# carlobaldassi/gimp-lqr-plugin

Hardware: AMD Instinct MI355X
Metric: Mseams*pixels/sec on 4K RGBA (higher is better)
Workload: dtype f32; 1 GPU; batch4k: 64 x 3840x2160 RGBA per GPU, resize to 3640x2160 (200 vertical seams each), side-switch 2; images_per_gpu=64, width=3840, height=2160, new_width=3640, new_height=2160, parallelism=images sharded i mod N, no data-path collective, streams_per_gpu=1

## Files before the change

gimp-lqr-plugin_amd/csrc/k_oneoff.hip:

```cpp
#include "lqr_common.h"
#include "lqr_kernels.h"

__global__ __launch_bounds__(256) void k_vs_commit(const DevCarver *cs, int w0, int h0, int wc0, int n_seams, int first_level,
                                                    int finish)
{
    const GCarver c = gview(cs[blockIdx.y]);
    extern __shared__ int smi[];
    int *xs = smi;
    int *lvl = smi + vsc_lvl_off(n_seams);
    __shared__ int s_wave[4];
    const int y = blockIdx.x, tid = threadIdx.x;
    for (int k = tid; k < n_seams; k += 256) xs[k] = c.seam_log[(size_t) k * h0 + y];
    for (int i = tid; i < wc0; i += 256) lvl[i] = 0;
    __syncthreads();
    for (int k = tid; k < n_seams; k += 256) {
        int pz = xs[k];
        for (int j = k - 1; j >= 0; j--) if (xs[j] <= pz) pz++;
        lvl[pz] = first_level + k;
    }
    __syncthreads();
    gi32 *vrow = c.vs + (size_t) y * w0;
    int carry = 0;
    for (int base = 0; base < w0; base += 256) {
        int col = base + tid;
        bool z = (col < w0) && (vrow[col] == 0);
        int total;
        int rank = carry + block_rank_256(z, s_wave, total);
        if (z) {
            int l = lvl[rank];
            if (l == 0 && finish) l = w0;
            if (l) vrow[col] = l;
        }
        carry += total;
    }
}

template <bool DEEP>
__global__ __launch_bounds__(256) void k_inflate(const InflateDev *jobs, int w0, int w1, int l, int max_level, int *dev_err)
{
    __shared__ int s_wave[4];
    extern __shared__ unsigned s_seen[];
    const int n_levels = l - max_level + 1, lvl0 = 2 * max_level - 1;
    for (int i = threadIdx.x; i < (n_levels + 31) / 32; i += 256) s_seen[i] = 0u;
    __syncthreads();
    bool twice = false;
    const InflateDev j = jobs[blockIdx.y];
    const uint8_t *rgb = j.rgb;
    const int32_t *vs = j.vs;
    const float *bias = j.bias, *rig = j.rig;
    uint8_t *nrgb = j.nrgb;
    int32_t *nvs = j.nvs;
    float *nbias = j.nbias, *nrig = j.nrig;
    const int ch = j.ch;
    const int y = blockIdx.x, tid = threadIdx.x;
    const int32_t *vrow = vs + (size_t) y * w0;
    const size_t ri = (size_t) y * w0, ro = (size_t) y * w1;
    int carry = 0;
    for (int base = 0; base < w0; base += 256) {
        int col = base + tid;
        int v = (col < w0) ? vrow[col] : 0;
        bool dup = (col < w0) && v != 0 && v <= l + max_level - 1 && v >= 2 * max_level - 1;
        if (dup) twice |= (atomicOr(&s_seen[(v - lvl0) >> 5], 1u << ((v - lvl0) & 31)) >> ((v - lvl0) & 31)) & 1u;
        int total;
        int rank = carry + block_rank_256(dup, s_wave, total);
        if (col < w0) {
            int z = col + rank;
            int left = col > 0 ? col - 1 : col;
            if (dup) {
                BasePx<DEEP>::avg(nrgb + (ro + z) * ch, rgb + (ri + left) * ch, rgb + (ri + col) * ch, ch, j.depth);
                if (nbias) nbias[ro + z] = __fmul_rn(__fadd_rn(bias[ri + left], bias[ri + col]), 0.5f);
                if (nrig) nrig[ro + z] = __fmul_rn(__fadd_rn(rig[ri + left], rig[ri + col]), 0.5f);
                if (nvs) nvs[ro + z] = l - v + max_level;
                z++;
            }
            BasePx<DEEP>::move(nrgb + (ro + z) * ch, rgb + (ri + col) * ch, ch);
            if (nbias) nbias[ro + z] = bias[ri + col];
            if (nrig) nrig[ro + z] = rig[ri + col];
            if (nvs) nvs[ro + z] = v ? v + l - max_level + 1 : 0;
        }
        carry += total;
    }
    if (dev_err && (twice || (tid == 0 && carry != n_levels))) dev_fail(dev_err, DEVERR_LEVELS);
}

__global__ __launch_bounds__(256) void k_vmap_check(const int32_t *map, int len, int depth, int *dev_err)
{
    extern __shared__ unsigned s_seen[];
    __shared__ int s_cnt;
    const int tid = threadIdx.x;
    for (int i = tid; i < (depth + 31) / 32; i += 256) s_seen[i] = 0u;
    if (tid == 0) s_cnt = 0;
    __syncthreads();
    const int32_t *row = map + (size_t) blockIdx.x * len;
    bool bad = false;
    int cnt = 0;
    for (int x = tid; x < len; x += 256) {
        const int v = row[x];
        if (v < 0 || v > depth) bad = true;
        else if (v) { bad |= (atomicOr(&s_seen[(v - 1) >> 5], 1u << ((v - 1) & 31)) >> ((v - 1) & 31)) & 1u; cnt++; }
    }
    for (int o = 32; o > 0; o >>= 1) cnt += __shfl_down(cnt, o);
    if ((tid & 63) == 0) atomicAdd(&s_cnt, cnt);
    __syncthreads();
    if (bad || (tid == 0 && s_cnt != depth)) dev_fail(dev_err, DEVERR_VMAP);
}

__global__ __launch_bounds__(256) void k_vmap_check_t(const int32_t *map, int32_t *out, int width, int height, int depth, int *dev_err)
{
    extern __shared__ unsigned s_seen[];
    __shared__ int32_t tile[VT_LINES][33];
    __shared__ int s_cnt[VT_LINES];
    const int tid = threadIdx.x, words = (depth + 31) / 32;
    const int col0 = blockIdx.x * VT_LINES;
    for (int i = tid; i < VT_LINES * words; i += 256) s_seen[i] = 0u;
    if (tid < VT_LINES) s_cnt[tid] = 0;
    bool bad = false;
    for (int row0 = 0; row0 < height; row0 += 32) {
        __syncthreads();
        for (int i = tid; i < VT_LINES * 32; i += 256) {
            const int r = i / VT_LINES, c = i % VT_LINES;
            if (row0 + r < height && col0 + c < width) tile[c][r] = map[(size_t) (row0 + r) * width + col0 + c];
        }
        __syncthreads();
        for (int i = tid; i < VT_LINES * 32; i += 256) {
            const int c = i / 32, r = i % 32;
            if (row0 + r < height && col0 + c < width) {
                const int v = tile[c][r];
                out[(size_t) (col0 + c) * height + row0 + r] = v;
                if (v < 0 || v > depth) bad = true;
                else if (v) {
                    bad |= (atomicOr(&s_seen[c * words + ((v - 1) >> 5)], 1u << ((v - 1) & 31)) >> ((v - 1) & 31)) & 1u;
                    atomicAdd(&s_cnt[c], 1);
                }
            }
        }
    }
    __syncthreads();
    if (tid < VT_LINES && col0 + tid < width && s_cnt[tid] != depth) bad = true;
    if (bad) dev_fail(dev_err, DEVERR_VMAP);
}

__global__ __launch_bounds__(256) void k_seam_check(const DevCarver *cs, int h, int wc0, int n_seams, int delta, int *dev_err)
{
    const GCarver c = gview_phys(cs[blockIdx.y]);
    const int y = blockIdx.x * 256 + threadIdx.x;
    if (y >= h) return;
    bool bad = false;
    for (int k = 0; k < n_seams; k++) {
        const int x = c.seam_log[(size_t) k * h + y];
        bad |= (x < 0) || (x >= wc0 - k);
        if (y > 0) { const int xu = c.seam_log[(size_t) k * h + y - 1]; bad |= (x - xu > delta) || (xu - x > delta); }
    }
    if (bad) dev_fail(dev_err, DEVERR_SEAMLOG);
}

__global__ __launch_bounds__(256) void k_vs_rollback(const DevCarver *cs, size_t n, int first_level, int finish_level)
{
    const GCarver c = gview_phys(cs[blockIdx.y]);
    for (size_t i = (size_t) blockIdx.x * 256 + threadIdx.x; i < n; i += (size_t) gridDim.x * 256) {
        const int v = c.vs[i];
        if (v >= first_level || (finish_level > 0 && v == finish_level)) c.vs[i] = 0;
    }
}

__global__ void k_inject(const DevCarver *cs, int what, int h, int w0, int log_index, int first_level)
{
    const GCarver c = gview_phys(cs[0]);
// ... 146 lines not shown
```

gimp-lqr-plugin_amd/csrc/lqr_kernels.h:

```cpp
#pragma once
#include "lqr_common.h"
#include "lqr_pixel.h"


template <class FORM> __global__ void k_wk_init(const DevCarver *cs, int w, int h, int stride, typename FORM::Arg a);
template <class FORM> __global__ __launch_bounds__(256) void k_wk_init_visible(const DevCarver *cs, int w0, int h, int stride, typename FORM::Arg a);
#define K_EMAP_FORMS(X) X(0, false) X(1, false) X(2, false) X(3, false) X(4, false) X(5, false) X(6, false) X(0, true) X(1, true) X(2, true) X(6, true)
#define K_EMAP_UPDATE_NT_FORMS(X, ...) X(12, __VA_ARGS__) X(36, __VA_ARGS__) X(68, __VA_ARGS__)
template <int NRG, bool VALUE> __global__ void k_emap_full(const DevCarver *cs, DpK p, int w, int h, int stride);
#define K_WK_INIT_EMAP_FORMS(X) X(0) X(1) X(2) X(3) X(4) X(5) X(6)
template <int NRG> __global__ __launch_bounds__(256) void k_wk_init_emap(const DevCarver *cs, DpK p, int w, int h, int stride);
__global__ void k_mask_add(float *plane, int w0, const uint8_t *mask, int channels, int mw, int x0, int y0, int x1, int y1,
                           int nx, int ny, int transposed, int is_rig, int bias_factor);
template <int NRG, int EU_NT, bool VALUE> __global__ __launch_bounds__(64) void k_emap_update(const DevCarver *cs, DpK p, int w, int h, int stride, int k, int epoch);
template <bool VALUE> __global__ __launch_bounds__(256) void k_frozen_catchup(const DevCarver *cs, int from, int to, int w_from, int h, int stride);

__global__ __launch_bounds__(VPATH_THREADS) void k_vpath(const DevCarver *cs, int w, int h, int stride, int lr, int delta, int log_index, int moved_unit);
#define K_VPATH1_FORMS(X) X(1) X(2) X(3) X(4) X(5) X(6) X(7)
#define K_VP_FORMS(X) K_VPATH1_FORMS(X) X(8) X(9) X(10)
template <int DELTA> __global__ __launch_bounds__(VPATH_THREADS) void k_vpath1(const DevCarver *cs, int w, int h, int stride, int lr, int log_index, int moved_unit);
unsigned long long *lqr_moved_bytes_dev(void);

template <int DELTA> __global__ __launch_bounds__(256) void k_vp_maps(const DevCarver *cs, int w, int h, int stride);
template <int DELTA> __global__ __launch_bounds__(VPATH_THREADS) void k_vp_solve(const DevCarver *cs, int w, int h, int stride, int lr, int log_index, int moved_unit);

__global__ __launch_bounds__(256) void k_carve(const DevCarver *cs, int w, int h, int stride, int delta, int move_dp);
#define K_CARVE_E_FORMS(X) X(0) X(1) X(2) X(3) X(4) X(5) X(6)
template <int NRG> __global__ __launch_bounds__(256) void k_carve_e(const DevCarver *cs, DpK p, int w, int h, int stride, int move_dp, int k, int epoch, int line);
#define K_CARVE_U_FORMS(X) X(0) X(1) X(2) X(3) X(4) X(5) X(6)
template <int NRG> __global__ __launch_bounds__(256) void k_carve_u(const DevCarver *cs, DpK p, int w, int h, int stride, int move_dp, int k, int epoch, int n, int line);
#define K_CARVE_V_DELTAS(X) X(1) X(2)
#define K_CARVE_V_FORMS(X) X(0, 1) X(1, 1) X(2, 1) X(3, 1) X(4, 1) X(5, 1) X(6, 1) X(0, 2) X(1, 2) X(2, 2) X(3, 2) X(4, 2) X(5, 2) X(6, 2)
template <int NRG, int DELTA> __global__ __launch_bounds__(256) __attribute__((amdgpu_waves_per_eu(5))) void k_carve_v(const DevCarver *cs, DpK p, int w, int h, int stride, int lr, int move_dp, int k, int epoch, int n,
                                                                                  int moved_unit, unsigned tag, unsigned long long *list, unsigned long long *moved_bytes, int *dev_err, int line);

#define K_DP_SWEEP_PXT_FORMS(X) X(1) X(2) X(4) X(8) X(16)
#define K_LR_RIG_FORMS(X) X(false, false) X(false, true) X(true, false) X(true, true)
template <int PXT, bool UPDATE, int NTH = DP_THREADS> __global__ __launch_bounds__(NTH) void k_dp_sweep(const DevCarver *cs, DpK p, int w, int h, int stride, int lr);
__global__ __launch_bounds__(64) void k_band_update(const DevCarver *cs, DpK p, int w, int h, int stride, int lr);
template <int PXL, int NW, int R, bool LR, bool RIG> __global__ __launch_bounds__(64 * NW) void k_band_update_mw(const DevCarver *cs, DpK p, int w, int h, int stride);
template <int NW, bool LR, bool RIG> __global__ __launch_bounds__(128 * NW) void k_band_update_tw(const DevCarver *cs, DpK p, int w, int h, int stride, int *dev_err);

template <bool LR, bool RIG> __global__ __launch_bounds__(64) void k_dp_tile(const DevCarver *cs, DpK p, int w, int h, int stride, int y0);
#define K_DP_TILE_P_FORMS_D(X, LR, UPD, D) X(GENERAL, 2, LR, false, UPD, D, false, 16) X(GENERAL, 2, LR, true, UPD, D, false, 16) X(GENERAL, 2, LR, true, UPD, D, true, 16)
#define K_DP_TILE_P_FORMS_W(X, LR, UPD, D) X(GENERAL, 2, LR, true, UPD, D, false, 16) X(GENERAL, 2, LR, true, UPD, D, true, 16)
#define K_DP_TILE_P_FORMS_LR(X, LR, UPD) \
    X(PX4, 4, LR, false, UPD, 1, false, 16) X(PX4, 4, LR, true, UPD, 1, false, 16) X(PLAIN, 2, LR, false, UPD, 1, false, 16) X(PLAIN, 2, LR, true, UPD, 1, false, 16) \
    X(GENERAL, 2, LR, true, UPD, 1, true, 16) K_DP_TILE_P_FORMS_D(X, LR, UPD, 2) K_DP_TILE_P_FORMS_D(X, LR, UPD, 3) K_DP_TILE_P_FORMS_D(X, LR, UPD, 4) \
    K_DP_TILE_P_FORMS_W(X, LR, UPD, 5) K_DP_TILE_P_FORMS_W(X, LR, UPD, 6) K_DP_TILE_P_FORMS_W(X, LR, UPD, 7) K_DP_TILE_P_FORMS_W(X, LR, UPD, 8) K_DP_TILE_P_FORMS_W(X, LR, UPD, 9) K_DP_TILE_P_FORMS_W(X, LR, UPD, 10)
#define K_DP_TILE_P_FORMS_24(X, UPD) X(PLAIN, 2, false, false, UPD, 1, false, 24) X(PLAIN, 2, false, true, UPD, 1, false, 24) X(PLAIN, 2, true, false, UPD, 1, false, 24) X(PLAIN, 2, true, true, UPD, 1, false, 24)
#define K_DP_TILE_P_FORMS(X) K_DP_TILE_P_FORMS_LR(X, false, false) K_DP_TILE_P_FORMS_LR(X, false, true) K_DP_TILE_P_FORMS_LR(X, true, false) K_DP_TILE_P_FORMS_LR(X, true, true) \
    K_DP_TILE_P_FORMS_24(X, false) K_DP_TILE_P_FORMS_24(X, true)
template <int PX, bool LR, bool RIG, bool UPDATE, int DELTA = 1, bool RIGM = false, int HLN = 16>
__global__ __launch_bounds__(64 * DPP_W) void k_dp_tile_p(DevCarver *cs, DpK p, int w, int h, int stride, unsigned long long *exch, int epoch, int *dev_err);

#define K_BAND_LEVELS_FORMS_D(X, LR, D) X(LR, false, D, false) X(LR, true, D, false) X(LR, true, D, true)
#define K_BAND_LEVELS_FORMS_W(X, LR, D) X(LR, true, D, false) X(LR, true, D, true)
#define K_BAND_LEVELS_FORMS_LR(X, LR) K_BAND_LEVELS_FORMS_D(X, LR, 1) K_BAND_LEVELS_FORMS_D(X, LR, 2) K_BAND_LEVELS_FORMS_D(X, LR, 3) K_BAND_LEVELS_FORMS_D(X, LR, 4) \
    K_BAND_LEVELS_FORMS_W(X, LR, 5) K_BAND_LEVELS_FORMS_W(X, LR, 6) K_BAND_LEVELS_FORMS_W(X, LR, 7) K_BAND_LEVELS_FORMS_W(X, LR, 8) K_BAND_LEVELS_FORMS_W(X, LR, 9) K_BAND_LEVELS_FORMS_W(X, LR, 10)
#define K_BAND_LEVELS_FORMS(X) K_BAND_LEVELS_FORMS_LR(X, false) K_BAND_LEVELS_FORMS_LR(X, true)
template <bool LR, bool RIG, int DELTA, bool RIGM>
__global__ __launch_bounds__(128) __attribute__((amdgpu_waves_per_eu(2, 2))) void k_band_levels(DevCarver *cs, DpK p, int w, int h, int stride, unsigned long long *exch, int epoch, int *dev_err, int P, int n_img, int store_rows);

#define K_BAND_LEVELS2_FORMS(X) X(false, false) X(false, true) X(true, false) X(true, true)
template <bool LR, bool RIG>
__global__ __launch_bounds__(256) __attribute__((amdgpu_waves_per_eu(2, 2))) void k_band_levels2(DevCarver *cs, DpK p, int w, int h, int stride, unsigned long long *exch, int epoch, int *dev_err, int P, int n_img, int store_rows);
void lqr_levels_report_rows(int on);
void lqr_levels2_debug(int v);
int lqr_levels2_stats(unsigned long long *out, int reset);

__global__ __launch_bounds__(256) void k_vs_commit(const DevCarver *cs, int w0, int h0, int wc0, int n_seams, int first_level, int finish);
template <bool DEEP> __global__ __launch_bounds__(256) void k_inflate(const InflateDev *jobs, int w0, int w1, int l, int max_level, int *dev_err);
__global__ __launch_bounds__(256) void k_vmap_check(const int32_t *map, int len, int depth, int *dev_err);
__global__ __launch_bounds__(256) void k_vmap_check_t(const int32_t *map, int32_t *out, int width, int height, int depth, int *dev_err);
__global__ __launch_bounds__(256) void k_seam_check(const DevCarver *cs, int h, int wc0, int n_seams, int delta, int *dev_err);
__global__ __launch_bounds__(256) void k_vs_rollback(const DevCarver *cs, size_t n, int first_level, int finish_level);
__global__ void k_inject(const DevCarver *cs, int what, int h, int w0, int log_index, int first_level);
template <bool DEEP> __global__ __launch_bounds__(256) void k_compact(const uint8_t *rgb, const int32_t *vs, const float *bias, const float *rig,
                                                  uint8_t *nrgb, float *nbias, float *nrig, int32_t *nvmap, int w0, int w, int ch, int level, int depth);
template <bool DEEP> __global__ __launch_bounds__(256) void k_compact_jobs(const InflateDev *jobs, int w0, int w, int level);
__global__ void k_transpose(const InflateDev *jobs, int w, int h);
__global__ void k_transpose_px(const InflateDev *jobs, int w, int h);
__global__ __launch_bounds__(256) void k_mask_line_max(const uint8_t *mask, int channels, int width, int a0, int b0, int line_len, int direction, int *out);

#define K_COMPACT_SIZES_FORMS(X) X(false) X(true)
#define K_TRANSPOSE_SIZES_FORMS(X) X(false) X(true)
template <bool DEEP> __global__ __launch_bounds__(256) void k_compact_sizes(const uint8_t *rgb, const int32_t *vs, const SizeJob *jobs, int n_jobs, int w0, int bytes);
template <bool WIDE> __global__ __launch_bounds__(256) void k_transpose_sizes(const SizeJob *jobs, int h, int bytes);

#define K_FWD_INIT_FORMS(X) X(0) X(1) X(2) X(3)
#define K_FWD_SEAM_FORMS(X) X(1) X(2) X(4) X(8) X(16)
template <int DEPTH> __global__ __launch_bounds__(256) void k_fwd_init(const FwdJob *jobs, int L, int H, int fw0, int strided, DeepRead rd, int w_start, int orientation);
template <int PXT> __global__ __launch_bounds__(FWD_THREADS) void k_fwd_seam(const FwdJob *jobs, int wc, int L, int H);
__global__ __launch_bounds__(FWD_REMOVE_THREADS) void k_fwd_remove(const FwdJob *jobs, int wc, int L, int H, int level, int orientation);

#define K_CLIP_SEAM_FORMS(X) X(1) X(2) X(4) X(8) X(16)
__global__ __launch_bounds__(CLIPFWD_FOLD_THREADS) void k_clip_fold(const FwdJob *jobs, const float *in, int first, int count, int last, int L, int H, int fw0, int strided,
                                                                   int w_start, float temporal, float *cost, float *pm);
template <int PXT> __global__ __launch_bounds__(FWD_THREADS) void k_clip_seam(const float *cost, int8_t *choice, int32_t *seam, int wc, int L, int H);
__global__ __launch_bounds__(FWD_REMOVE_THREADS) void k_clip_remove(float *cost, uint16_t *pos, const int32_t *seam, int32_t *map, int wc, int L, int H, int level, int orientation);
__global__ __launch_bounds__(CLIPFWD_REFRESH_THREADS) void k_clip_refresh(const float *in, int n, float *cost, const uint16_t *pos, const int32_t *seam, int wn, int L, int H);

#define K_STATIC_FOLD_FORMS(X) X(0, 0, true) X(1, 0, true) X(2, 0, true) X(6, 0, true) X(0, 0, false) X(1, 0, false) X(2, 0, false) X(6, 0, false) \
    X(0, 1, false) X(1, 1, false) X(2, 1, false) X(6, 1, false) X(0, 2, false) X(1, 2, false) X(2, 2, false) X(6, 2, false) \
    X(0, 3, false) X(1, 3, false) X(2, 3, false) X(6, 3, false)
template <int NRG, int DEPTH, bool PACKED>
__global__ __launch_bounds__(STATIC_THREADS) void k_static_fold(const StaticFrame *frames, int count, int first, int W, int H, int transposed, int orientation, DeepRead rd,
                                                     float alpha, float *s_plane, float *t_plane, float *i_plane, float *e_out);

__global__ __launch_bounds__(DISCARD_THREADS) void k_discard_line(const float *bias, const int32_t *vs, int w0, float thr, int level, int depth, int *res);
__global__ __launch_bounds__(DISCARD_THREADS) void k_discard_cross(const float *bias, const int32_t *vs, int w0, int h0, float thr, int level, int depth,
                                                                 int *partial, int *res);
__global__ __launch_bounds__(DISCARD_THREADS) void k_discard_rank(const float *bias, const int32_t *vs, int w0, int w, float thr, int level, int depth, int *col,
                                                                int *res);
__global__ __launch_bounds__(DISCARD_THREADS) void k_discard_fold(const int *partial, int w0, int tiles, int *res);

template <class T> __global__ __launch_bounds__(256) void k_mask_add_f(float *plane, int w0, const T *mask, int mw, int x0, int y0, int x1, int y1, int nx, int ny,
                                                                       int transposed, int is_rig, int bias_factor);
__global__ __launch_bounds__(256) void k_mask_scatter(float *plane, const int *index, const double *value, size_t n, int is_rig);
__global__ __launch_bounds__(256) void k_plane_transpose(const float *plane, float *out, int w0, int h0);

template <bool PIC> __global__ __launch_bounds__(256) void k_energy_range(const DevCarver *cs, int w, int h, int stride, float *partials);
__global__ __launch_bounds__(256) void k_energy_plane(const DevCarver *cs, int w, int h, int stride, int transposed, int normalised,
                                                      const float *partials, int n_partials, float *out);
#define K_ENERGY_OUT_FORMS_T(X, T) X(T, 0) X(T, 1) X(T, 2) X(T, 3)
#define K_ENERGY_OUT_FORMS(X) K_ENERGY_OUT_FORMS_T(X, 0) K_ENERGY_OUT_FORMS_T(X, 1) K_ENERGY_OUT_FORMS_T(X, 2) K_ENERGY_OUT_FORMS_T(X, 3) K_ENERGY_OUT_FORMS_T(X, 4) K_ENERGY_OUT_FORMS_T(X, 5) K_ENERGY_OUT_FORMS_T(X, 6)
template <int TYPE, int DEPTH> __global__ __launch_bounds__(256) void k_energy_out(const DevCarver *cs, int w, int h, int stride, int transposed,
                                                                                    const float *partials, int n_partials, uint8_t *out);
```

gimp-lqr-plugin_amd/csrc/lqr_shim.hip:

```cpp
#include "lqr_common.h"
#include "lqr_kernels.h"
#include "lqr_own.h"
#include "lqr_pool.h"
#include "lqr_stage.h"
#include <atomic>
#include <memory>
#include <dirent.h>

static thread_local std::string g_err;
static int g_device = -1;

static int *g_dev_err_host = nullptr;
static int *g_dev_err = nullptr;

#define HIPCK_VOID(expr) do { hipError_t e__ = (expr); if (e__ != hipSuccess) { g_err = std::string(#expr) + ": " + hipGetErrorString(e__); (void) hipGetLastError(); } } while (0)
#define HIPCK(expr)                                                                   \
    do {                                                                              \
        hipError_t e__ = (expr);                                                      \
        if (e__ != hipSuccess) {                                                      \
            g_err = std::string(#expr) + ": " + hipGetErrorString(e__);               \
            (void) hipGetLastError();                                                 \
            return (e__ == hipErrorOutOfMemory) ? LQRHIP_ENOMEM : LQRHIP_EHIP;        \
        }                                                                             \
    } while (0)

static PlanKnobs g_knobs;
static PlanDevice g_dev;

namespace {
struct WorkingPlanes {
    DevBuf<uint32_t> pix;
    DevBuf<float> en, m, m2, bias, rig;
    DevBuf<int8_t> least, least2;
    DevBuf<int32_t> seam_x, seam_log, flags;
    DevBuf<int8_t> vp_map, vp_path;
};
}
struct __attribute__((visibility("hidden"))) LqrHipCarver {
    int ch = 0;
    int depth = 0;
    int luma = 0;
    int mode = RD_RGB, alpha = -1, black = -1;
    int pix_deep = 0;
    int w0 = 0, h0 = 0;
    DevBuf<uint8_t> rgb0;
    DevBuf<int32_t> vs;
    DevBuf<float> bias0, rig0;
    int active = 0;
    int stride = 0, wk_h = 0;
    WorkingPlanes wk;
    int log_cap = 0, log_h = 0;
    int frozen_epoch = 0;
    int owed_to = 0, owed_w = 0, owed_h = 0;
    LqrHipCarver *root = nullptr;
    std::vector<LqrHipCarver *> aux;
    LqrHipBatch *batch = nullptr;
};

static inline size_t px_bytes(const LqrHipCarver *c) { return (size_t) c->ch << (c->depth == 0 ? 0 : c->depth == 1 ? 1 : c->depth == 2 ? 2 : 3); }
static inline int32_t *vs_of(const LqrHipCarver *c) { return (c->root ? c->root : c)->vs; }

namespace {
struct PlaneJob {
    LqrHipCarver *c;
    DevBuf<uint8_t> nrgb;
    DevBuf<float> nbias, nrig;
};
}
struct PlaneJobs {
    std::vector<PlaneJob> jobs;
    std::vector<DevBuf<int32_t>> new_vs;
    std::vector<InflateDev> dev;
    DevBuf<InflateDev> d_dev;
    size_t n_narrow = 0;
    int add(LqrHipCarver *c, const int32_t *vs_old, int32_t *nvs, size_t n1)
    {
        jobs.push_back(PlaneJob{c, {}, {}, {}});
        PlaneJob &j = jobs.back();
        int rc = j.nrgb.alloc(n1 * px_bytes(c), "&j.nrgb");
        if (!rc && c->bias0) rc = j.nbias.alloc(n1, "&j.nbias");
        if (!rc && c->rig0) rc = j.nrig.alloc(n1, "&j.nrig");
        if (rc) return rc;
        dev.push_back(InflateDev{c->rgb0, vs_old, c->bias0, c->rig0, j.nrgb, nvs, j.nbias, j.nrig, (int) px_bytes(c), c->depth});
        return 0;
    }
    int stage(hipStream_t s, bool by_width)
    {
        n_narrow = std::stable_partition(dev.begin(), dev.end(), [&](const InflateDev &d) { return d.ch <= 4 && (by_width || d.depth == 0); }) - dev.begin();
        int rc = d_dev.alloc(dev.size(), "&d_dev");
        if (rc) return rc;
        HIPCK(hipMemcpyAsync(d_dev, dev.data(), dev.size() * sizeof(InflateDev), hipMemcpyHostToDevice, s));
        return 0;
    }
    size_t n_wide() const { return dev.size() - n_narrow; }
    const InflateDev *d_wide() const { return d_dev + n_narrow; }
};
static void commit(PlaneJobs &pj)
{
    for (auto &j : pj.jobs) {
        j.c->rgb0 = std::move(j.nrgb);
        if (j.nbias) j.c->bias0 = std::move(j.nbias);
        if (j.nrig) j.c->rig0 = std::move(j.nrig);
    }
}

struct PendingInflate { PlaneJobs pj; int kind = 0 , w1 = 0, h1 = 0; };

struct LqrHipBatch {
    std::vector<LqrHipCarver *> cs;
    DevCarver *d_desc = nullptr;
    size_t desc_cap = 0;
    hipStream_t stream = nullptr;
    DevBuf<unsigned long long> exch;
    int exch_ntiles = 0, exch_n = 0, exch_px = 0;
    int tile_epoch = 0;
    DevBuf<unsigned long long> wlist;
    unsigned wlist_launches = 0;
    bool dirty = true;
    int shared_n = 1;
    bool shared = false;
    bool safe = false;
    std::unique_ptr<PendingInflate> pending_inflate;
};
static bool g_no_spin = false;

struct ProfRec {
    std::vector<std::pair<hipEvent_t, hipEvent_t>> ev;
    double bytes = 0;
};
static int g_prof = 0;
static std::map<std::string, ProfRec> g_profrec;
static hipStream_t g_stream0 = nullptr;
static unsigned long long g_census[LQRHIP_CENSUS_SLOTS];
#define CENSUS(slot) (g_census[(slot)]++)
extern "C" int lqrhip_launch_census(unsigned long long *out, int n, int reset)
{
// ... 216 lines not shown
        const unsigned hw = std::thread::hardware_concurrency();
        return new StageRing(dev, STAGE_SLOTS, (size_t) 4 << 20, hw >= 16 ? 8 : hw >= 4 ? (int) hw / 2 : 1);
    }();
    return *ring;
}
static int h2d_staged(void *dst, const void *src, size_t bytes) { return stage_ring().upload(dst, src, bytes); }
static int d2h_staged(void *dst, const void *src, size_t bytes) { return stage_ring().download(dst, src, bytes); }

static inline bool reads_value(const LqrHipCarver *c)
{
    if (c->depth != 0 || c->ch > 4 || (c->mode != RD_GREY && c->mode != RD_RGB)) return true;
    return c->black >= 0 || c->alpha != (c->ch == 2 ? 1 : c->ch == 4 ? 3 : -1);
}
static inline DeepRead deep_read(const LqrHipCarver *c) { return DeepRead{c->ch, c->mode, c->alpha, c->black, c->luma}; }
template <class F> static inline void with_form(const LqrHipCarver *c, F f)
{
    if (reads_value(c)) f(std::true_type{}); else f(std::false_type{});
}
constexpr int plane_nrg(bool value, int nrg) { return value && nrg >= 3 && nrg <= 5 ? nrg - 3 : nrg; }
static inline int nrg_index(int nrg_func) { return nrg_func >= 0 && nrg_func <= 5 ? nrg_func : 6; }
static int no_form(const char *family) { g_err = std::string(family) + ": no instantiation for the parameters asked for"; return LQRHIP_EARG; }
#define LISTED_CASE_(N) if (v__ == N) { f__(std::integral_constant<int, N>{}); return true; }
#define with_listed(LIST, v, f) [&](int v__, auto f__) { LIST(LISTED_CASE_) return false; }(v, f)
static void default_read(LqrHipCarver *c)
{
    c->mode = c->ch <= 2 ? RD_GREY : c->ch <= 4 ? RD_RGB : c->ch == 5 ? RD_CMYK : RD_CUSTOM;
    c->alpha = c->ch == 2 ? 1 : c->ch == 4 ? 3 : c->ch == 5 ? 4 : -1;
    c->black = c->ch == 5 ? 3 : -1;
}

static int batch_sync_of(LqrHipCarver *c)
{
    LqrHipCarver *r = c->root ? c->root : c;
    if (r->batch) HIPCK(hipStreamSynchronize(r->batch->stream));
    return 0;
}

extern "C" LqrHipCarver *lqrhip_carver_create_ext(const void *rgb, int w, int h, int channels, int depth)
{
    if (depth < 0 || depth > 3 || channels < 1 || channels > LQRHIP_MAX_CHANNELS) { g_err = "unsupported colour depth / channels"; return nullptr; }
    if (lqrhip_init() < 0) return nullptr;
    LqrHipCarver *c = new LqrHipCarver();
    c->ch = channels; c->depth = depth; c->w0 = w; c->h0 = h;
    default_read(c);
    const size_t n = (size_t) w * h, bytes = n * px_bytes(c);
    if (c->rgb0.alloc(bytes, "&c->rgb0") || c->vs.alloc(n, "&c->vs")) { lqrhip_carver_destroy(c); return nullptr; }
    if (hipMemsetAsync(c->vs, 0, n * sizeof(int32_t), g_stream0) != hipSuccess || h2d_staged(c->rgb0, rgb, bytes) != 0) {
        g_err = "upload failed";
        lqrhip_carver_destroy(c);
        return nullptr;
    }
    return c;
}

extern "C" LqrHipCarver *lqrhip_carver_create(const unsigned char *rgb, int w, int h, int channels)
{
    return lqrhip_carver_create_ext(rgb, w, h, channels, 0);
}

extern "C" int lqrhip_carver_set_read_luma(LqrHipCarver *c, int luma)
{
    const int changed = reads_value(c) && (luma != 0) != (c->luma != 0);
    c->luma = luma != 0;
    return changed;
}

extern "C" int lqrhip_carver_set_read(LqrHipCarver *c, int image_type, int alpha, int black)
{
    static const int mode_of[8] = {RD_RGB, RD_RGB, RD_GREY, RD_GREY, RD_CMY, RD_CMYK, RD_CMYK, RD_CUSTOM};
    if (image_type < 0 || image_type > 7 || alpha >= c->ch || black >= c->ch) return LQRHIP_EARG;
    const bool was = reads_value(c);
    const int mode = mode_of[image_type], a = alpha < 0 ? -1 : alpha, k = black < 0 ? -1 : black;
    const bool differs = mode != c->mode || a != c->alpha || k != c->black;
    c->mode = mode; c->alpha = a; c->black = k;
    return (differs && (was || reads_value(c))) ? 1 : 0;
}

static inline void drop_catchup(LqrHipCarver *c)
{
    c->owed_to = 0; c->owed_w = 0; c->owed_h = 0;
    c->frozen_epoch = 0;
}

static void free_working(LqrHipCarver *c)
{
    c->wk = WorkingPlanes();
    c->log_cap = 0; c->log_h = 0;
    drop_catchup(c);
}

extern "C" void lqrhip_carver_destroy(LqrHipCarver *c)
{
    if (!c) return;
    {
        LqrHipCarver *r = c->root ? c->root : c;
        if (r->batch && r->batch->stream) (void) hipStreamSynchronize(r->batch->stream);
        if (c->batch && c->batch != r->batch && c->batch->stream) (void) hipStreamSynchronize(c->batch->stream);
        if (g_stream0) (void) hipStreamSynchronize(g_stream0);
        (void) hipGetLastError();
    }
    delete c;
}

extern "C" int lqrhip_carver_attach(LqrHipCarver *root, LqrHipCarver *aux)
{
    if (root->w0 != aux->w0 || root->h0 != aux->h0) return LQRHIP_EARG;
    aux->vs.reset();
    aux->root = root;
    root->aux.push_back(aux);
    if (root->batch) root->batch->dirty = true;
    return 0;
}

static int ensure_working(LqrHipCarver *c, int w, int h)
{
    int stride = plane_stride(w);
    bool need_bias = c->bias0 != nullptr, need_rig = c->rig0 != nullptr;
    const int deep = reads_value(c) ? 1 : 0;
    WorkingPlanes &k = c->wk;
    if (k.pix && c->stride == stride && c->wk_h == h && (!!k.bias == need_bias) && (!!k.rig == need_rig) && c->pix_deep == deep) return 0;
    free_working(c);
    c->stride = 0; c->wk_h = 0;
    size_t n = plane_elems(stride, h);
    const size_t npix = deep ? 2 * n : n;
    int rc;
    if ((rc = k.pix.alloc(npix, "&c->pix")) || (rc = k.en.alloc(n, "&c->en")) || (rc = k.m.alloc(n, "&c->m")) || (rc = k.least.alloc(n, "&c->least")) ||
        (rc = k.seam_x.alloc(seam_x_elems(h), "&c->seam_x")) || (rc = k.flags.alloc((size_t) FLAG_WORDS, "&c->flags")) ||
        (need_bias && (rc = k.bias.alloc(n, "&c->bias"))) || (need_rig && (rc = k.rig.alloc(n, "&c->rig")))) {
        free_working(c);
        return rc;
    }
    hipError_t e = hipMemsetAsync(k.least, 0, n, g_stream0);
    if (e == hipSuccess) e = hipMemsetAsync(k.m, 0, n * sizeof(float), g_stream0);
    if (e == hipSuccess) e = hipMemsetAsync(k.en, 0, n * sizeof(float), g_stream0);
    if (e == hipSuccess) e = hipMemsetAsync(k.pix, 0, npix * sizeof(uint32_t), g_stream0);
    if (e == hipSuccess) e = hipMemsetAsync(k.flags, 0, (size_t) FLAG_WORDS * sizeof(int32_t), g_stream0);
    if (e == hipSuccess) e = hipStreamSynchronize(g_stream0);
    if (e != hipSuccess) { free_working(c); HIPCK(e); }
    c->stride = stride; c->wk_h = h; c->pix_deep = deep;
    if (c->batch) c->batch->dirty = true;
    return 0;
}

static int ensure_log(LqrHipCarver *c, int n_seams, int h)
{
    if (c->wk.seam_log && c->log_cap >= n_seams && c->log_h == h) return 0;
    int rc = c->wk.seam_log.alloc(seam_log_elems(n_seams, h), "&c->seam_log");
    if (rc) return rc;
    c->log_cap = n_seams; c->log_h = h;
    if (c->batch) c->batch->dirty = true;
    return 0;
}

extern "C" int lqrhip_carver_activate(LqrHipCarver *c)
{
    c->active = 1;
    return ensure_working(c, c->w0, c->h0);
}

extern "C" int lqrhip_mask_plane_ensure(LqrHipCarver *c, int is_rigmask)
{
    DevBuf<float> &plane = is_rigmask ? c->rig0 : c->bias0;
    if (plane) return 0;
    int rc = batch_sync_of(c);
    if (rc) return rc;
    const size_t n = (size_t) c->w0 * c->h0;
    if ((rc = plane.alloc(n, "plane"))) return rc;
    hipError_t e = dzero(plane, n * sizeof(float));
    if (e != hipSuccess) { plane.reset(); HIPCK(e); }
    if (c->batch) c->batch->dirty = true;
    return 0;
}

extern "C" int lqrhip_mask_add(LqrHipCarver *c, const unsigned char *mask, int channels, int width, int height, int x_off,
                               int y_off, int transposed, int is_rigmask, int bias_factor)
{
    int rc = batch_sync_of(c);
    if (rc) return rc;
    if ((rc = lqrhip_mask_plane_ensure(c, is_rigmask))) return rc;
    float *plane = is_rigmask ? c->rig0 : c->bias0;
    const MaskClip k = mask_clip(c->w0, c->h0, width, height, x_off, y_off, transposed);
    if (k.nx <= 0 || k.ny <= 0) return 0;
    const size_t mbytes = (size_t) width * height * channels;
    Scratch tmp(g_stream0);
    uint8_t *dmask = tmp.get<uint8_t>(mbytes, "&dmask", rc);
    if (rc || (rc = h2d_staged(dmask, mask, mbytes))) return rc;
    dim3 grid(tiles_of(k.nx, 256), k.ny);
    hipLaunchKernelGGL(k_mask_add, grid, dim3(256), 0, g_stream0, plane, c->w0, dmask, channels, width, k.x0, k.y0, k.x1, k.y1, k.nx, k.ny,
                       transposed, is_rigmask, bias_factor);
    HIPCK(hipGetLastError());
    HIPCK(hipStreamSynchronize(g_stream0));
    tmp.done();
    return 0;
}

extern "C" int lqrhip_mask_add_f(LqrHipCarver *c, const void *mask, int depth, int on_device, int width, int height, int x_off, int y_off,
                                 int transposed, int is_rigmask, int bias_factor)
{
    if ((depth != 2 && depth != 3) || !mask || width < 1 || height < 1) { g_err = "mask: float or double values, at least 1 x 1"; return LQRHIP_EARG; }
    int rc = batch_sync_of(c);
    if (rc) return rc;
    if ((rc = lqrhip_mask_plane_ensure(c, is_rigmask))) return rc;
    float *plane = is_rigmask ? c->rig0 : c->bias0;
    const MaskClip k = mask_clip(c->w0, c->h0, width, height, x_off, y_off, transposed);
    if (k.nx <= 0 || k.ny <= 0) return 0;
    const size_t mbytes = (size_t) width * height * (depth == 2 ? sizeof(float) : sizeof(double));
    Scratch tmp(g_stream0);
    const void *src = mask;
    if (!on_device) {
        uint8_t *staged = tmp.get<uint8_t>(mbytes, "&staged", rc);
        if (rc || (rc = h2d_staged(staged, mask, mbytes))) return rc;
        src = staged;
    }
    dim3 grid(tiles_of(k.nx, 256), k.ny);
    if (depth == 2)
        hipLaunchKernelGGL(k_mask_add_f<float>, grid, dim3(256), 0, g_stream0, plane, c->w0, (const float *) src, width, k.x0, k.y0, k.x1, k.y1, k.nx, k.ny,
                           transposed, is_rigmask, bias_factor);
    else
        hipLaunchKernelGGL(k_mask_add_f<double>, grid, dim3(256), 0, g_stream0, plane, c->w0, (const double *) src, width, k.x0, k.y0, k.x1, k.y1, k.nx, k.ny,
                           transposed, is_rigmask, bias_factor);
    HIPCK(hipGetLastError());
    HIPCK(hipStreamSynchronize(g_stream0));
    tmp.done();
    return 0;
}

static unsigned long long g_mask_flushes = 0;
extern "C" unsigned long long lqrhip_debug_mask_flushes(void) { return g_mask_flushes; }

extern "C" int lqrhip_mask_scatter(LqrHipCarver *c, int is_rigmask, const int *index, const double *value, const size_t *start, int buckets)
{
    if (buckets < 1 || start[buckets] == 0) return 0;
    int rc = batch_sync_of(c);
    if (rc) return rc;
    if ((rc = lqrhip_mask_plane_ensure(c, is_rigmask))) return rc;
    float *plane = is_rigmask ? c->rig0 : c->bias0;
    const size_t n = start[buckets];
    Scratch tmp(g_stream0);
    int *dindex = tmp.get<int>(n, "&dindex", rc);
    if (rc) return rc;
    double *dvalue = tmp.get<double>(n, "&dvalue", rc);
    if (rc || (rc = h2d_staged(dindex, index, n * sizeof(int))) || (rc = h2d_staged(dvalue, value, n * sizeof(double)))) return rc;
    for (int b = 0; b < buckets; b++) {
        const size_t nb = start[b + 1] - start[b];
        if (!nb) continue;
        hipLaunchKernelGGL(k_mask_scatter, dim3((unsigned) blocks_of(nb, 256)), dim3(256), 0, g_stream0, plane, dindex + start[b], dvalue + start[b],
                           nb, is_rigmask);
        HIPCK(hipGetLastError());
        g_mask_flushes++;
    }
    HIPCK(hipStreamSynchronize(g_stream0));
    tmp.done();
    return 0;
}

extern "C" int lqrhip_mask_clear(LqrHipCarver *c, int is_rigmask)
{
    DevBuf<float> &plane = is_rigmask ? c->rig0 : c->bias0;
    if (!plane) return 0;
    int rc = batch_sync_of(c);
    if (rc) return rc;
    HIPCK(hipStreamSynchronize(g_stream0));
    plane.reset();
    if (c->batch) c->batch->dirty = true;
    return 0;
}

extern "C" int lqrhip_read_mask_plane(LqrHipCarver *c, int is_rigmask, int transposed, float *out)
{
    int rc = batch_sync_of(c);
    if (rc) return rc;
    const size_t n = (size_t) c->w0 * c->h0;
    const float *plane = is_rigmask ? c->rig0 : c->bias0;
    if (!plane) { memset(out, 0, n * sizeof(float)); return 0; }
    if (!transposed) return d2h_staged(out, plane, n * sizeof(float));
    Scratch tmp(g_stream0);
    float *t = tmp.get<float>(n, "&t", rc);
    if (rc) return rc;
    hipLaunchKernelGGL(k_plane_transpose, dim3(tiles_of(c->w0, 16), tiles_of(c->h0, 16)), dim3(256), 0, g_stream0, plane, t, c->w0, c->h0);
    hipError_t e = hipGetLastError();
    if (e != hipSuccess) { g_err = std::string("k_plane_transpose: ") + hipGetErrorString(e); return LQRHIP_EHIP; }
    if ((rc = d2h_staged(out, t, n * sizeof(float)))) return rc;
    (void) hipStreamSynchronize(g_stream0);
    tmp.done();
    return 0;
}

extern "C" void lqrhip_set_sub_batches(int n) { g_knobs.sub_batches = n > 0 ? n : 0; }
extern "C" int lqrhip_sub_batches(int n)
{
    const char *q = getenv("GPU_MAX_HW_QUEUES");
    g_dev.hw_queues = q ? atoi(q) : 0;
    return plan_streams(g_knobs, g_dev, n);
}

extern "C" void lqrhip_batch_set_shared(LqrHipBatch *b, int shared) { b->shared = shared != 0; b->shared_n = shared > 1 ? shared : 1; }
extern "C" void lqrhip_batch_set_safe(LqrHipBatch *b, int safe) { b->safe = safe != 0; if (safe) g_fault_stats[6]++; }

static const size_t MAX_PARKED = 4;
static std::vector<hipStream_t> g_parked_streams;
static unsigned long long g_fixed_stats[3];
static std::multimap<size_t, DevCarver *> g_parked_desc;
extern "C" void lqrhip_debug_fixedcost(unsigned long long out4[4], int reset)
{
    out4[0] = g_parked_streams.size();
    for (int i = 0; i < 3; i++) out4[i + 1] = g_fixed_stats[i];
    if (reset) memset(g_fixed_stats, 0, sizeof g_fixed_stats);
}
static void unpark_all(void)
{
    for (hipStream_t s : g_parked_streams) (void) hipStreamDestroy(s);
    g_parked_streams.clear();
    for (auto &kv : g_parked_desc) (void) hipFree(kv.second);
    g_parked_desc.clear();
}

extern "C" LqrHipBatch *lqrhip_batch_create(LqrHipCarver **carvers, int n)
{
    if (lqrhip_init() < 0 || n <= 0) return nullptr;
    LqrHipBatch *b = new LqrHipBatch();
    for (int i = 0; i < n; i++) {
        b->cs.push_back(carvers[i]);
        carvers[i]->batch = b;
    }
    hipError_t e = hipSuccess;
    if (!g_parked_streams.empty()) { b->stream = g_parked_streams.back(); g_parked_streams.pop_back(); g_fixed_stats[0]++; }
    else e = hipStreamCreateWithFlags(&b->stream, hipStreamNonBlocking);
    if (e == hipSuccess) {
        auto it = g_parked_desc.lower_bound((size_t) n);
        if (it != g_parked_desc.end()) { b->d_desc = it->second; b->desc_cap = it->first; g_parked_desc.erase(it); }
        else if ((e = hipMalloc((void **) &b->d_desc, sizeof(DevCarver) * n)) == hipSuccess) b->desc_cap = (size_t) n;
    }
    if (e != hipSuccess) {
        g_err = "batch_create failed";
        (void) hipGetLastError();
        if (b->stream) (void) hipStreamDestroy(b->stream);
        for (auto *c : b->cs) if (c->batch == b) c->batch = nullptr;
        delete b;
        return nullptr;
    }
    g_live_batches.push_back(b);
    return b;
}

static void invalidate_all_batches(void)
{
    for (auto *b : g_live_batches) { b->exch_ntiles = 0; b->dirty = true; }
}

extern "C" void lqrhip_batch_abort(LqrHipBatch *b)
{
    if (!b) return;
    (void) hipStreamSynchronize(b->stream);
    (void) hipGetLastError();
// ... 59 lines not shown

struct ProfScope {
    ProfRec *rec = nullptr;
    hipEvent_t e0 = nullptr, e1 = nullptr;
    hipStream_t s;
    ProfScope(const char *name, hipStream_t stream, double bytes) : s(stream)
    {
        if (!g_prof || (g_prof == 2 && strcmp(name, "carve") != 0)) return;
        rec = &g_profrec[name];
        rec->bytes += bytes;
        (void) hipEventCreate(&e0); (void) hipEventCreate(&e1);
        (void) hipEventRecord(e0, s);
    }
    ~ProfScope()
    {
        if (!rec) return;
        (void) hipEventRecord(e1, s);
        rec->ev.emplace_back(e0, e1);
    }
};

extern "C" void lqrhip_prof_enable(int on) { g_prof = on; }
extern "C" void lqrhip_prof_reset(void)
{
    for (auto &kv : g_profrec) for (auto &e : kv.second.ev) { (void) hipEventDestroy(e.first); (void) hipEventDestroy(e.second); }
    g_profrec.clear();
}
extern "C" int lqrhip_prof_get(const char *kernel, double *ms_total, long long *launches, double *bytes_total)
{
    auto it = g_profrec.find(kernel);
    *ms_total = 0; *launches = 0; *bytes_total = 0;
    if (it == g_profrec.end()) return 0;
    (void) hipDeviceSynchronize();
    for (auto &e : it->second.ev) {
        float ms = 0;
        if (hipEventElapsedTime(&ms, e.first, e.second) == hipSuccess) *ms_total += ms;
    }
    *launches = (long long) it->second.ev.size();
    *bytes_total = it->second.bytes;
    return 0;
}

extern "C" int lqrhip_prof_get_union(const char *kernel, double *ms_union)
{
    *ms_union = 0;
    auto it = g_profrec.find(kernel);
    if (it == g_profrec.end() || it->second.ev.empty()) return 0;
    (void) hipDeviceSynchronize();
    const hipEvent_t base = it->second.ev[0].first;
    std::vector<std::pair<float, float>> iv;
    for (auto &e : it->second.ev) {
        float a = 0, b = 0;
        if (hipEventElapsedTime(&a, base, e.first) != hipSuccess) { (void) hipGetLastError(); float t = 0; if (hipEventElapsedTime(&t, e.first, base) == hipSuccess) a = -t; else (void) hipGetLastError(); }
        if (hipEventElapsedTime(&b, base, e.second) != hipSuccess) { (void) hipGetLastError(); float t = 0; if (hipEventElapsedTime(&t, e.second, base) == hipSuccess) b = -t; else (void) hipGetLastError(); }
        iv.emplace_back(a, b);
    }
    std::sort(iv.begin(), iv.end());
    float end = -1e30f;
    for (auto &p : iv) {
        if (p.first > end) { *ms_union += p.second - p.first; end = p.second; }
        else if (p.second > end) { *ms_union += p.second - end; end = p.second; }
    }
    return 0;
}

static int pay_catchup(LqrHipBatch *b);
static int wk_init_prepare(LqrHipBatch *b)
{
    LqrHipCarver *c0 = b->cs[0];
    int w = c0->w0, h = c0->h0, rc;
    for (auto *c : b->cs) {
        if (c->w0 != w || c->h0 != h || c->ch != c0->ch || c->depth != c0->depth || c->luma != c0->luma || c->mode != c0->mode ||
            c->alpha != c0->alpha || c->black != c0->black)
            return LQRHIP_EARG;
        if ((rc = ensure_working(c, w, h))) return rc;
    }
    if ((rc = batch_upload(b))) return rc;
    for (auto *c : b->cs) drop_catchup(c);
    return 0;
}
extern "C" int lqrhip_wk_init(LqrHipBatch *b, int from_visible)
{
    LqrHipCarver *c0 = b->cs[0];
    int w = c0->w0, h = c0->h0, rc;
    if ((rc = wk_init_prepare(b))) return rc;
    const dim3 grid(tiles_of(c0->stride, 256), h, (unsigned) b->cs.size()), grid_v(h, (unsigned) b->cs.size());
#define LAUNCH_WK(FORM, arg) do { if (from_visible) hipLaunchKernelGGL(k_wk_init_visible<FORM>, grid_v, dim3(256), 0, b->stream, b->d_desc, w, h, c0->stride, arg); \
                                  else hipLaunchKernelGGL(k_wk_init<FORM>, grid, dim3(256), 0, b->stream, b->d_desc, w, h, c0->stride, arg); } while (0)
    if (!reads_value(c0)) LAUNCH_WK(PixPacked, c0->ch);
    else if (c0->depth == 0) LAUNCH_WK(PixValue<0>, deep_read(c0));
    else if (c0->depth == 1) LAUNCH_WK(PixValue<1>, deep_read(c0));
    else if (c0->depth == 2) LAUNCH_WK(PixValue<2>, deep_read(c0));
    else LAUNCH_WK(PixValue<3>, deep_read(c0));
#undef LAUNCH_WK
    HIPCK(hipGetLastError());
    return 0;
}

extern "C" int lqrhip_emap_build(LqrHipBatch *b, const LqrHipDpParams *p, int w, int h)
{
    int rc;
    if ((rc = pay_catchup(b))) return rc;
    if ((rc = batch_upload(b))) return rc;
    LqrHipCarver *c0 = b->cs[0];
    dim3 grid(tiles_of(w, 256), h, (unsigned) b->cs.size());
    DpK k = make_dpk(p, c0->ch);
    const bool value = reads_value(c0);
    const int nrg = plane_nrg(value, nrg_index(p->nrg_func));
#define CASE(N, V) if (nrg == N && value == V) hipLaunchKernelGGL((k_emap_full<N, V>), grid, dim3(256), 0, b->stream, b->d_desc, k, w, h, c0->stride); else
    K_EMAP_FORMS(CASE) return no_form("k_emap_full");
#undef CASE
    HIPCK(hipGetLastError());
    return 0;
}

extern "C" int lqrhip_wk_init_emap(LqrHipBatch *b, const LqrHipDpParams *p, int w, int h)
{
    LqrHipCarver *c0 = b->cs[0];
    int rc;
    if (reads_value(c0) || w != c0->w0 || h != c0->h0) return (rc = lqrhip_wk_init(b, 0)) ? rc : lqrhip_emap_build(b, p, w, h);
    if ((rc = wk_init_prepare(b))) return rc;
    const dim3 grid(tiles_of(tiles_of(c0->stride, 4), 256), h, (unsigned) b->cs.size());
    DpK k = make_dpk(p, c0->ch);
    const int nrg = nrg_index(p->nrg_func);
#define CASE(N) if (nrg == N) hipLaunchKernelGGL(k_wk_init_emap<N>, grid, dim3(256), 0, b->stream, b->d_desc, k, w, h, c0->stride); else
    K_WK_INIT_EMAP_FORMS(CASE) return no_form("k_wk_init_emap");
#undef CASE
    HIPCK(hipGetLastError());
    return 0;
}

extern "C" int lqrhip_energy_out(LqrHipBatch *b, int w, int h, int transposed, int form, int depth, int image_type, void *out, int on_device)
{
    static const int channels_of[7] = {3, 4, 1, 2, 3, 4, 5};
    if (b->cs.size() != 1 || !out || w < 1 || h < 1 || form < 0 || form > 2) { g_err = "energy read-out: one carver, a buffer, form 0 .. 2"; return LQRHIP_EARG; }
    if (form != 2) { depth = 2; image_type = 2; }
    if (depth < 0 || depth > 3 || image_type < 0 || image_type > 6) { g_err = "energy read-out: depth 0 .. 3, image type 0 .. 6"; return LQRHIP_EARG; }
    int rc;
    if ((rc = batch_upload(b))) return rc;
    LqrHipCarver *c0 = b->cs[0];
    if (!c0->wk.en) return LQRHIP_EARG;
    const size_t bytes = (size_t) w * h * channels_of[image_type] << depth;
    const int chunks = (w + EO_CHUNK - 1) / EO_CHUNK;
    const int n_partials = form ? (int) std::min((long long) EO_MAX_PARTIALS, (long long) h * chunks) : 0;
    Scratch tmp(b->stream);
    float *partials = form ? tmp.get<float>((size_t) 2 * n_partials, "&partials", rc) : nullptr;
    if (rc) return rc;
    uint8_t *staged = on_device ? nullptr : tmp.get<uint8_t>(bytes, "&staged", rc);
    if (rc) return rc;
    uint8_t *dst = on_device ? (uint8_t *) out : staged;
    {
        ProfScope prof("energy_out", b->stream, (double) w * h * sizeof(float) * (form ? 2 : 1) + (double) bytes);
        if (form == 1) hipLaunchKernelGGL(k_energy_range<false>, dim3(n_partials), dim3(256), 0, b->stream, b->d_desc, w, h, c0->stride, partials);
        if (form == 2) hipLaunchKernelGGL(k_energy_range<true>, dim3(n_partials), dim3(256), 0, b->stream, b->d_desc, w, h, c0->stride, partials);
        const int W = transposed ? h : w, H = transposed ? w : h;
        const dim3 grid((W + EO_TILE - 1) / EO_TILE, (H + EO_TILE - 1) / EO_TILE);
#define CASE(T, D) if (image_type == T && depth == D) hipLaunchKernelGGL((k_energy_out<T, D>), grid, dim3(256), 0, b->stream, b->d_desc, w, h, c0->stride, transposed, partials, n_partials, dst); else
        if (form != 2)
            hipLaunchKernelGGL(k_energy_plane, grid, dim3(256), 0, b->stream, b->d_desc, w, h, c0->stride, transposed, form, partials, n_partials, (float *) dst);
        else K_ENERGY_OUT_FORMS(CASE) return no_form("k_energy_out");
#undef CASE
    }
    hipError_t e = hipGetLastError();
    if (e == hipSuccess) e = hipStreamSynchronize(b->stream);
    if (e != hipSuccess) { g_err = std::string("energy read-out: ") + hipGetErrorString(e); (void) hipGetLastError(); return LQRHIP_EHIP; }
    if ((rc = check_dev_error())) return rc;
    if (!on_device && (rc = d2h_staged(out, staged, bytes))) return rc;
    tmp.done();
    return 0;
}

static int launch_dp_tiled(LqrHipBatch *b, const DpK &k, int w, int h, int lr)
{
    LqrHipCarver *c0 = b->cs[0];
    const dim3 grid(tiles_of(w, DPT_OWN), (unsigned) b->cs.size());
    for (int y0 = 0; y0 < h; y0 += DPT_ROWS) {
        CENSUS(LQRHIP_CENSUS_DP_TILE);
#define CASE(LRV, RIGV) if ((lr != 0) == LRV && (k.use_rig != 0) == RIGV) hipLaunchKernelGGL((k_dp_tile<LRV, RIGV>), grid, dim3(64), 0, b->stream, b->d_desc, k, w, h, c0->stride, y0); else
        K_LR_RIG_FORMS(CASE) return no_form("k_dp_tile");
#undef CASE
    }
    HIPCK(hipGetLastError());
    return 0;
}

extern "C" void lqrhip_set_vpath_mode(int mode, int par_max) { g_knobs.vpath_mode = mode; if (par_max > 0) g_knobs.vpath_par_max = par_max; }
extern "C" void lqrhip_set_sweep_threads(int n) { g_knobs.sweep_threads = n == 256 ? 256 : DP_THREADS; }
extern "C" void lqrhip_set_carve_fused(int max_images) { g_knobs.carve_fused = max_images == 1 ? 4 : max_images < 0 ? 0 : max_images; }
extern "C" void lqrhip_set_carve_beside(int mode) { g_knobs.carve_beside = mode < 0 ? -1 : mode ? 1 : 0; }
static unsigned long long g_carve_beside_launches;
extern "C" unsigned long long lqrhip_carve_beside_launches(int reset)
{
    const unsigned long long v = g_carve_beside_launches;
    if (reset) g_carve_beside_launches = 0;
    return v;
}
extern "C" void lqrhip_set_backtrack_beside(int mode) { g_knobs.backtrack_beside = mode < 0 ? -1 : mode ? 1 : 0; }
static unsigned long long g_backtrack_beside_launches;
extern "C" unsigned long long lqrhip_backtrack_beside_launches(int reset)
{
    const unsigned long long v = g_backtrack_beside_launches;
    if (reset) g_backtrack_beside_launches = 0;
// ... 321 lines not shown
        if (int rc = launch_band_levels(b, k, wnew, h, leftright_next, s.levels_P, s.levels_wg_slots, s.levels_store, v.rigm)) return rc;
    } else if (s.band == LQRHIP_CENSUS_BAND_TW) {
        ProfScope ps("band_update", b->stream, 0);
        CENSUS(LQRHIP_CENSUS_BAND_TW);
#define CASE(LRV, RIGV) if ((leftright_next != 0) == LRV && (k.use_rig != 0) == RIGV) hipLaunchKernelGGL((k_band_update_tw<4, LRV, RIGV>), dim3(n), dim3(128 * 4), band_tw_lds(h), b->stream, b->d_desc, k, wnew, h, stride, g_dev_err); else
        K_LR_RIG_FORMS(CASE) return no_form("k_band_update_tw");
#undef CASE
    } else if (s.band == LQRHIP_CENSUS_BAND_MW8 || s.band == LQRHIP_CENSUS_BAND_MW16) {
        ProfScope ps("band_update", b->stream, 0);
        const int nw = s.band == LQRHIP_CENSUS_BAND_MW16 ? 16 : 8;
        CENSUS(nw == 16 ? LQRHIP_CENSUS_BAND_MW16 : LQRHIP_CENSUS_BAND_MW8);
#define CASE_NW(NWV, LRV, RIGV) if (nw == NWV && (leftright_next != 0) == LRV && (k.use_rig != 0) == RIGV) hipLaunchKernelGGL((k_band_update_mw<2, NWV, 8, LRV, RIGV>), dim3(n), dim3(64 * NWV), band_mw_lds(h), b->stream, b->d_desc, k, wnew, h, stride); else
#define CASE(LRV, RIGV) CASE_NW(8, LRV, RIGV) CASE_NW(16, LRV, RIGV)
        K_LR_RIG_FORMS(CASE) return no_form("k_band_update_mw");
#undef CASE
#undef CASE_NW
    } else {
        ProfScope ps("band_update", b->stream, 0);
        CENSUS(LQRHIP_CENSUS_BAND_GENERIC);
        hipLaunchKernelGGL(k_band_update, dim3(n), dim3(64), 0, b->stream, b->d_desc, k, wnew, h, stride, leftright_next);
    }
    ProfScope ps("dp_update", b->stream, 0);
    return launch_dp<true>(b, k, s.dp, v.rigm, wnew, h, leftright_next);
}

static int seam_step_impl(LqrHipBatch *b, const LqrHipDpParams *p, int w, int h, int log_index, int leftright_pick,
                          int full_rebuild, int leftright_next)
{
    int rc;
    LqrHipCarver *c0 = b->cs[0];
    for (auto *c : b->cs)
        if (log_index >= c->log_cap || c->owed_to) return LQRHIP_EARG;
    if ((rc = batch_upload(b))) return rc;
    const PlanBatch pb = plan_batch(b);
    const StepPlan s = plan_seam_step(g_knobs, g_dev, pb, p->delta_x, p->use_rigidity != 0, w, h, full_rebuild != 0, log_index + 1 - c0->frozen_epoch);
    const int wnew = w - 1, move_dp = (wnew > 1 && !full_rebuild) ? 1 : 0;
    const int moved_unit = 2 * (4 + (move_dp ? 5 : 0) + (pb.rigmask ? 4 : 0));
    StepVals v{make_dpk(p, c0->ch), w, h, c0->stride, log_index, leftright_pick, leftright_next, move_dp, moved_unit, c0->frozen_epoch,
               pb.value, pb.rigm(p->use_rigidity != 0), (unsigned) b->cs.size()};
    if ((rc = launch_backtrack(b, s, v)) || (rc = launch_carve(b, s, v))) return rc;
    if (s.dp.form < 0) { HIPCK(hipGetLastError()); return 0; }
    if ((rc = launch_energy(b, s, v))) return rc;
    if (s.full || s.band < 0) {
        ProfScope ps(s.full ? "dp_sweep" : "dp_update_tiled", b->stream, s.full ? 9.0 * wnew * h * v.n : 0);
        rc = s.full ? launch_dp<false>(b, v.k, s.dp, v.rigm, wnew, h, leftright_next) : launch_dp<true>(b, v.k, s.dp, v.rigm, wnew, h, leftright_next);
    } else rc = launch_band(b, s, v);
    if (rc) return rc;
    HIPCK(hipGetLastError());
    return 0;
}

extern "C" int lqrhip_seam_step(LqrHipBatch *b, const LqrHipDpParams *p, int w, int h, int log_index, int leftright_pick,
                                int full_rebuild, int leftright_next)
{
    const int rc = seam_step_impl(b, p, w, h, log_index, leftright_pick, full_rebuild, leftright_next);
    if (rc == 0) inject_after_step(b, h, log_index);
    static const char *dump = getenv("LQRHIP_DUMP");
    if (rc == 0 && dump) {
        static int call = 0;
        LqrHipCarver *c = b->cs[0];
        HIPCK(hipStreamSynchronize(b->stream));
        const size_t np = (size_t) c->stride * h;
        std::vector<int> hdr = {w, h, c->stride, log_index, FLAG_COUNT}, flags(FLAG_COUNT), seam(h);
        std::vector<float> m(np);
        std::vector<int8_t> least(np);
        HIPCK(hipMemcpy(flags.data(), c->wk.flags, FLAG_COUNT * sizeof(int), hipMemcpyDeviceToHost));
        HIPCK(hipMemcpy(seam.data(), c->wk.seam_x, (size_t) h * sizeof(int), hipMemcpyDeviceToHost));
        HIPCK(hipMemcpy(m.data(), c->wk.m, np * sizeof(float), hipMemcpyDeviceToHost));
        HIPCK(hipMemcpy(least.data(), c->wk.least, np, hipMemcpyDeviceToHost));
        char path[512];
        snprintf(path, sizeof path, "%s_%04d.bin", dump, call++);
        if (FILE *f = fopen(path, "wb")) {
            fwrite(hdr.data(), sizeof(int), hdr.size(), f); fwrite(flags.data(), sizeof(int), flags.size(), f);
            fwrite(seam.data(), sizeof(int), seam.size(), f); fwrite(m.data(), sizeof(float), np, f); fwrite(least.data(), 1, np, f);
            fclose(f);
        }
    }
    return rc;
}

extern "C" int lqrhip_seam_log_reserve(LqrHipBatch *b, int n_seams, int h)
{
    int rc;
    if ((rc = pay_catchup(b))) return rc;
    for (auto *c : b->cs) if ((rc = ensure_log(c, n_seams, h))) return rc;
    return 0;
}

extern "C" int lqrhip_vs_commit(LqrHipBatch *b, int w0, int h0, int wc0, int n_seams, int first_level, int finish)
{
    int rc;
    if ((rc = batch_upload(b))) return rc;
    size_t lds = vsc_lds(n_seams, wc0);
    if (lds > VSC_LDS_MAX) { g_err = "vs_commit: session too large for LDS"; return LQRHIP_EARG; }
    if (lds_needs_attr(lds)) {
        HIPCK(hipFuncSetAttribute((const void *) k_vs_commit, hipFuncAttributeMaxDynamicSharedMemorySize, (int) lds));
        CENSUS(LQRHIP_CENSUS_LDS_ATTR_COMMIT);
    }
    hipLaunchKernelGGL(k_vs_commit, dim3(h0, (unsigned) b->cs.size()), dim3(256), lds, b->stream, b->d_desc, w0, h0, wc0, n_seams,
                       first_level, finish);
    HIPCK(hipGetLastError());
    inject_after_commit(b, w0, h0, first_level);
    for (auto *c : b->cs) {
        if (c->frozen_epoch < n_seams) { c->owed_to = n_seams; c->owed_w = wc0 - n_seams; c->owed_h = h0; }
        else drop_catchup(c);
    }
    return 0;
}

static int g_selfcheck = 1, g_recovery = 1;
extern "C" void lqrhip_set_selfcheck(int on) { g_selfcheck = on != 0; }
extern "C" void lqrhip_set_recovery(int on) { g_recovery = on != 0; }
extern "C" int lqrhip_get_recovery(void) { return g_recovery; }
extern "C" int lqrhip_session_check(LqrHipBatch *b, int h, int wc0, int n_seams, int delta_x)
{
    int rc;
    if (!g_selfcheck || n_seams < 1) return 0;
    if ((rc = batch_upload(b))) return rc;
    hipLaunchKernelGGL(k_seam_check, dim3(tiles_of(h, 256), (unsigned) b->cs.size()), dim3(256), 0, b->stream, b->d_desc, h, wc0, n_seams, delta_x, g_dev_err);
    HIPCK(hipGetLastError());
    return 0;
}
extern "C" int lqrhip_session_rollback(LqrHipBatch *b, int w0, int h0, int first_level, int finish)
{
    (void) hipStreamSynchronize(b->stream);
    b->pending_inflate.reset();
    (void) hipGetLastError();
    if (g_dev_err_host) *g_dev_err_host = 0;
    invalidate_all_batches();
    int rc;
    if ((rc = batch_upload(b))) return rc;
    const size_t n = (size_t) w0 * h0;
    hipLaunchKernelGGL(k_vs_rollback, dim3((unsigned) std::min<size_t>(blocks_of(n, 256), 4096), (unsigned) b->cs.size()), dim3(256), 0, b->stream, b->d_desc, n, first_level, finish ? w0 : 0);
    HIPCK(hipGetLastError());
    HIPCK(hipStreamSynchronize(b->stream));
    for (auto *c : b->cs) drop_catchup(c);
    g_fault_stats[4]++;
    return 0;
}
static int g_inject_kind = 0, g_inject_step = 0, g_inject_times = 0;
extern "C" void lqrhip_debug_inject(int kind, int at_step, int times) { g_inject_kind = kind; g_inject_step = at_step; g_inject_times = kind ? std::max(times, 1) : 0; }
static void inject_after_step(LqrHipBatch *b, int h, int log_index)
{
    if (g_inject_times <= 0 || log_index != g_inject_step) return;
    if (g_inject_kind == 1 || g_inject_kind == 2) { *g_dev_err_host = g_inject_kind == 1 ? DEVERR_TILE_TIMEOUT : DEVERR_BAND_PREDICTION; }
    else if (g_inject_kind == 3 || g_inject_kind == 4) hipLaunchKernelGGL(k_inject, dim3(1), dim3(64), 0, b->stream, b->d_desc, g_inject_kind - 3, h, 0, log_index, 0);
    else return;
    g_inject_times--; g_fault_stats[5]++;
}
static void inject_after_commit(LqrHipBatch *b, int w0, int h0, int first_level)
{
    if (g_inject_times <= 0 || (g_inject_kind != 5 && g_inject_kind != 6)) return;
    if (g_inject_step > 0) { g_inject_step--; return; }
    hipLaunchKernelGGL(k_inject, dim3(1), dim3(64), 0, b->stream, b->d_desc, g_inject_kind - 3, h0, w0, 0, first_level);
    g_inject_times--; g_fault_stats[5]++;
}

namespace {
struct Staging {
    LqrHipBatch *b;
    bool keep = false;
    Staging(LqrHipBatch *batch, int kind, int w1, int h1) : b(batch)
    {
        b->pending_inflate.reset(new PendingInflate());
        b->pending_inflate->kind = kind; b->pending_inflate->w1 = w1; b->pending_inflate->h1 = h1;
    }
    ~Staging() { if (!keep) { lqr_stream_wait(b->stream); b->pending_inflate.reset(); } }
    PlaneJobs &jobs() const { return b->pending_inflate->pj; }
    int kept() { keep = true; return 0; }
};
}
static int inflate_stage(LqrHipBatch *b, int w0, int h0, int l, int max_level, const int32_t *levels)
{
    int rc;
    const int w1 = w0 + l - max_level + 1;
    Staging st(b, 0, w1, h0);
    PlaneJobs &pj = st.jobs();
    for (auto *c : b->cs) {
        pj.new_vs.emplace_back();
        DevBuf<int32_t> &nvs = pj.new_vs.back();
        if ((rc = nvs.alloc((size_t) w1 * h0, "&nvs"))) return rc;
        const int32_t *vs = levels ? levels : c->vs.get();
        for (auto *a : c->aux)
            if ((rc = pj.add(a, vs, nullptr, (size_t) w1 * h0))) return rc;
        if ((rc = pj.add(c, vs, nvs, (size_t) w1 * h0))) return rc;
    }
    if ((rc = pj.stage(b->stream, false))) return rc;
    const size_t lds = inflate_lds(l, max_level);
    if (pj.n_narrow)
        hipLaunchKernelGGL(k_inflate<false>, dim3(h0, (unsigned) pj.n_narrow), dim3(256), lds, b->stream, pj.d_dev.get(), w0, w1, l, max_level, g_selfcheck ? g_dev_err : (int *) nullptr);
    if (pj.n_wide())
        hipLaunchKernelGGL(k_inflate<true>, dim3(h0, (unsigned) pj.n_wide()), dim3(256), lds, b->stream, pj.d_wide(), w0, w1, l, max_level, g_selfcheck ? g_dev_err : (int *) nullptr);
    HIPCK(hipGetLastError());
    HIPCK(hipStreamSynchronize(b->stream));
    if ((rc = check_dev_error())) return rc;
    return st.kept();
}
extern "C" int lqrhip_inflate(LqrHipBatch *b, int w0, int h0, int l, int max_level) { return inflate_stage(b, w0, h0, l, max_level, nullptr); }

struct __attribute__((visibility("hidden"))) LqrHipVMap {
    DevBuf<int32_t> own;
    const int32_t *plane = nullptr;
    int len = 0, lines = 0, depth = 0;
};
extern "C" int lqrhip_vmap_stage(const int *map, int on_device, int width, int height, int depth, int orientation, LqrHipVMap **out)
{
    *out = nullptr;
    if (lqrhip_init() < 0) return LQRHIP_EHIP;
    const int len = orientation ? height : width, lines = orientation ? width : height;
    if (!map || width < 1 || height < 1 || (orientation != 0 && orientation != 1) || depth < 1 || depth >= len || depth >= LQRHIP_MAX_FRAME_WIDTH) {
        g_err = "vmap: depth, size or orientation out of range";
        return LQRHIP_EARG;
    }
    int rc;
    const size_t n = (size_t) width * height;
    std::unique_ptr<LqrHipVMap> m(new LqrHipVMap());
    m->len = len; m->lines = lines; m->depth = depth;
    Scratch tmp(g_stream0);
    const int32_t *src = (const int32_t *) map;
    if (!on_device) {
        int32_t *d = orientation ? tmp.get<int32_t>(n, "&vmap_raw", rc) : ((rc = m->own.alloc(n, "&vmap")) ? nullptr : m->own.get());
        if (rc) return rc;
        if ((rc = h2d_staged(d, map, n * sizeof(int32_t)))) return rc;
        src = d;
    }
    if (orientation) {
        if ((rc = m->own.alloc(n, "&vmap_t"))) return rc;
        const size_t lds = vmap_check_t_lds(depth);
        if (vmap_t_needs_attr(lds)) HIPCK(hipFuncSetAttribute((const void *) k_vmap_check_t, hipFuncAttributeMaxDynamicSharedMemorySize, (int) lds));
        hipLaunchKernelGGL(k_vmap_check_t, dim3(vmap_t_blocks(width)), dim3(256), lds, g_stream0, src, m->own.get(), width, height, depth, g_dev_err);
        m->plane = m->own;
    } else {
        hipLaunchKernelGGL(k_vmap_check, dim3(height), dim3(256), vmap_check_lds(depth), g_stream0, src, width, depth, g_dev_err);
        m->plane = src;
    }
    HIPCK(hipGetLastError());
    HIPCK(hipStreamSynchronize(g_stream0));
    tmp.done();
    if (g_dev_err_host && *g_dev_err_host == DEVERR_VMAP) {
        *g_dev_err_host = 0;
        g_err = "vmap: a value outside [0, depth], or a level that is missing or occurs twice in a line";
        return LQRHIP_EMAP;
    }
    if ((rc = check_dev_error())) return rc;
    *out = m.release();
    return 0;
}
extern "C" void lqrhip_vmap_release(LqrHipVMap *m) { delete m; }
extern "C" int lqrhip_vmap_load(LqrHipBatch *b, const LqrHipVMap *m)
{
    if (!m || !m->plane) return LQRHIP_EARG;
    for (auto *c : b->cs)
        if (c->w0 != m->len || c->h0 != m->lines) { g_err = "vmap: the carver's frame is not the map's"; return LQRHIP_EARG; }
    return inflate_stage(b, m->len, m->lines, m->depth, 1, m->plane);
}
extern "C" int lqrhip_planes_commit(LqrHipBatch *b)
{
    PendingInflate *pi = b->pending_inflate.get();
    if (!pi) return LQRHIP_EARG;
    PlaneJobs &pj = pi->pj;
    commit(pj);
    for (auto &j : pj.jobs) { j.c->w0 = pi->w1; j.c->h0 = pi->h1; }
    if (pi->kind != 0)
        for (auto *c : b->cs) drop_catchup(c);
    if (pi->kind != 2) {
        size_t i = 0;
        for (auto *c : b->cs) c->vs = std::move(pj.new_vs[i++]);
    }
    b->dirty = true;
    b->pending_inflate.reset();
    return 0;
}
extern "C" int lqrhip_inflate_commit(LqrHipBatch *b) { return lqrhip_planes_commit(b); }

extern "C" int lqrhip_flatten(LqrHipBatch *b, int w0, int h0, int w, int level)
{
    int rc;
    Staging st(b, 1, w, h0);
    PlaneJobs &pj = st.jobs();
    for (auto *c : b->cs) {
        pj.new_vs.emplace_back();
        DevBuf<int32_t> &nvs = pj.new_vs.back();
        if ((rc = nvs.alloc((size_t) w * h0, "&nvs"))) return rc;
        HIPCK(hipMemsetAsync(nvs, 0, (size_t) w * h0 * sizeof(int32_t), b->stream));
        for (auto *a : c->aux)
            if ((rc = pj.add(a, c->vs, nullptr, (size_t) w * h0))) return rc;
        if ((rc = pj.add(c, c->vs, nullptr, (size_t) w * h0))) return rc;
    }
    if ((rc = pj.stage(b->stream, true))) return rc;
    if (pj.n_narrow)
        hipLaunchKernelGGL(k_compact_jobs<false>, dim3(h0, (unsigned) pj.n_narrow), dim3(256), 0, b->stream, pj.d_dev.get(), w0, w, level);
    if (pj.n_wide())
        hipLaunchKernelGGL(k_compact_jobs<true>, dim3(h0, (unsigned) pj.n_wide()), dim3(256), 0, b->stream, pj.d_wide(), w0, w, level);
    HIPCK(hipGetLastError());
    HIPCK(hipStreamSynchronize(b->stream));
    return st.kept();
}

extern "C" int lqrhip_transpose(LqrHipBatch *b, int w, int h)
{
    int rc;
    Staging st(b, 2, h, w);
    PlaneJobs &pj = st.jobs();
    for (auto *c : b->cs) {
        for (auto *a : c->aux)
            if ((rc = pj.add(a, nullptr, nullptr, (size_t) w * h))) return rc;
        if ((rc = pj.add(c, nullptr, nullptr, (size_t) w * h))) return rc;
        HIPCK(hipMemsetAsync(c->vs, 0, (size_t) w * h * sizeof(int32_t), b->stream));
    }
    if ((rc = pj.stage(b->stream, true))) return rc;
    if (pj.n_narrow)
        hipLaunchKernelGGL(k_transpose, dim3(tiles_of(w, 32), tiles_of(h, 32), (unsigned) pj.n_narrow), dim3(32, 8), 0, b->stream, pj.d_dev.get(), w, h);
    if (pj.n_wide())
        hipLaunchKernelGGL(k_transpose_px, dim3(tiles_of(w, 32), tiles_of(h, 32), (unsigned) pj.n_wide()), dim3(32, 8), 0, b->stream, pj.d_wide(), w, h);
    HIPCK(hipGetLastError());
    HIPCK(hipStreamSynchronize(b->stream));
    return st.kept();
}

static void launch_read_visible(const LqrHipCarver *c, int w0, int h0, int w, int level, uint8_t *d)
{
#define LAUNCH_RV(DEEP) hipLaunchKernelGGL(k_compact<DEEP>, dim3(h0), dim3(256), 0, g_stream0, c->rgb0.get(), vs_of(c), (const float *) nullptr, (const float *) nullptr, \
                                           d, (float *) nullptr, (float *) nullptr, (int32_t *) nullptr, w0, w, (int) px_bytes(c), level, 0)
    if (px_bytes(c) > 4) LAUNCH_RV(true); else LAUNCH_RV(false);
#undef LAUNCH_RV
}
extern "C" int lqrhip_read_visible(LqrHipCarver *c, int w0, int h0, int w, int level, unsigned char *out)
{
    int rc = batch_sync_of(c);
    if (rc) return rc;
    size_t n = (size_t) w * h0 * px_bytes(c);
    Scratch tmp(g_stream0);
    uint8_t *d = tmp.get<uint8_t>(n, "&d", rc);
    if (rc) return rc;
    launch_read_visible(c, w0, h0, w, level, d);
    HIPCK(hipGetLastError());
    if ((rc = d2h_staged(out, d, n))) return rc;
    tmp.done();
    return 0;
}

extern "C" int lqrhip_read_visible_device(LqrHipCarver *c, int w0, int h0, int w, int level, void *device_out)
{
    int rc = batch_sync_of(c);
    if (rc) return rc;
    launch_read_visible(c, w0, h0, w, level, (uint8_t *) device_out);
    HIPCK(hipGetLastError());
    HIPCK(hipStreamSynchronize(g_stream0));
    return 0;
}

static const size_t SZ_SCRATCH_MAX = (size_t) 512 << 20;
extern "C" int lqrhip_read_sizes(LqrHipCarver *c, int w0, int h0, int transposed, const int *levels, int n, void *const *outs, int on_device)
{
    int rc = batch_sync_of(c);
    if (rc) return rc;
    if (n < 1 || !levels || !outs || w0 < 1 || h0 < 1) return LQRHIP_EARG;
    for (int k = 0; k < n; k++)
        if (levels[k] < 1 || levels[k] > w0 || !outs[k]) return LQRHIP_EARG;
    const size_t bytes = px_bytes(c);
    const int planes = (on_device ? 0 : 1) + (transposed ? 1 : 0);
    auto width_of = [&](int k) { return w0 - levels[k] + 1; };
    auto plane_bytes = [&](int k) { return ((size_t) width_of(k) * h0 * bytes + 255) & ~(size_t) 255; };
    struct Chunk { int first, count; };
    std::vector<Chunk> chunks;
    size_t scratch_bytes = 0;
    for (int k = 0; k < n;) {
        size_t used = 0;
        int m = 0;
        while (k + m < n && m < SZ_MAX_JOBS && (m == 0 || used + planes * plane_bytes(k + m) <= SZ_SCRATCH_MAX)) used += planes * plane_bytes(k + m), m++;
        chunks.push_back(Chunk{k, m});
        scratch_bytes = std::max(scratch_bytes, used);
        k += m;
    }
    std::vector<SizeJob> jobs(2 * (size_t) n);
    std::vector<const uint8_t *> result(n);
    Scratch tmp(g_stream0);
    SizeJob *d_jobs = tmp.get<SizeJob>(2 * (size_t) n, "&d_jobs", rc);
    if (rc) return rc;
    uint8_t *scratch = nullptr;
    if (planes) {
        scratch = tmp.get<uint8_t>(scratch_bytes, "&scratch", rc);
        if (rc) return rc;
    }
    for (const Chunk &ch : chunks) {
        size_t at = 0;
        for (int k = ch.first; k < ch.first + ch.count; k++) {
            uint8_t *frame = (uint8_t *) outs[k], *image = (uint8_t *) outs[k];
            if (planes) { frame = scratch + at; at += plane_bytes(k); }
            if (transposed && !on_device) { image = scratch + at; at += plane_bytes(k); }
            jobs[k] = SizeJob{frame, nullptr, levels[k], width_of(k)};
            jobs[n + k] = SizeJob{image, frame, levels[k], width_of(k)};
            result[k] = transposed ? image : frame;
        }
    }
    HIPCK(hipMemcpyAsync(d_jobs, jobs.data(), jobs.size() * sizeof(SizeJob), hipMemcpyHostToDevice, g_stream0));
    for (const Chunk &ch : chunks) {
#define LAUNCH_CS(DEEP) hipLaunchKernelGGL(k_compact_sizes<DEEP>, dim3(h0), dim3(256), 0, g_stream0, (const uint8_t *) c->rgb0.get(), (const int32_t *) vs_of(c), \
                                           (const SizeJob *) (d_jobs + ch.first), ch.count, w0, (int) bytes)
        if (bytes > 4) LAUNCH_CS(true); else LAUNCH_CS(false);
#undef LAUNCH_CS
        CENSUS(LQRHIP_CENSUS_COMPACT_SIZES);
        HIPCK(hipGetLastError());
        if (transposed) {
            int wmax = 0;
            for (int k = ch.first; k < ch.first + ch.count; k++) wmax = std::max(wmax, width_of(k));
            const dim3 grid(tiles_of(wmax, 32), tiles_of(h0, 32), (unsigned) ch.count);
#define LAUNCH_TS(WIDE) hipLaunchKernelGGL(k_transpose_sizes<WIDE>, grid, dim3(256), 0, g_stream0, (const SizeJob *) (d_jobs + n + ch.first), h0, (int) bytes)
            if (bytes > 4) LAUNCH_TS(true); else LAUNCH_TS(false);
#undef LAUNCH_TS
            CENSUS(LQRHIP_CENSUS_TRANSPOSE_SIZES);
            HIPCK(hipGetLastError());
        }
        if (!on_device)
            for (int k = ch.first; k < ch.first + ch.count; k++)
                if ((rc = d2h_staged(outs[k], result[k], (size_t) width_of(k) * h0 * bytes))) return rc;
    }
    HIPCK(hipStreamSynchronize(g_stream0));
    tmp.done();
    return 0;
}

static unsigned long long g_discard_launches[4];
extern "C" void lqrhip_discard_launches(unsigned long long out4[4], int reset)
{
    if (out4) memcpy(out4, g_discard_launches, sizeof g_discard_launches);
    if (reset) memset(g_discard_launches, 0, sizeof g_discard_launches);
}
extern "C" int lqrhip_discard_scan(LqrHipCarver *c, int w0, int h0, int w, int level, int depth, float strength, int which, int *out)
{
    if (!c || c->root || !out || w0 < 1 || h0 < 1 || w < 1 || w > w0 || level < 1 || depth < 0 || !(which & 3) || !(strength >= 0.0f) || c->w0 != w0 || c->h0 != h0) {
        g_err = "discard scan: a root carver in its own base layout, a level, a strength >= 0 and a scan to run";
        return LQRHIP_EARG;
    }
    int rc = batch_sync_of(c);
    if (rc) return rc;
    const bool line = which & LQRHIP_DISCARD_LINE, cross = which & LQRHIP_DISCARD_CROSS;
    memset(out, 0, discard_result_elems() * sizeof(int));
    if (!c->bias0) return 0;
    Scratch tmp(g_stream0);
    int *res = tmp.get<int>(discard_result_elems(), "&res", rc);
    if (rc) return rc;
    const bool ranked = cross && level > 1;
    int *partial = nullptr;
    if (cross) {
        partial = tmp.get<int>(ranked ? discard_rank_elems(w) : discard_partial_elems(w0, h0), "&partial", rc);
        if (rc) return rc;
    }
    HIPCK(hipMemsetAsync(res, 0, discard_result_elems() * sizeof(int), g_stream0));
    if (ranked) HIPCK(hipMemsetAsync(partial, 0, discard_rank_elems(w) * sizeof(int), g_stream0));
    const float thr = -strength;
    const double plane_bytes = 8.0 * w0 * h0;
    if (line) {
        ProfScope ps("discard_line", g_stream0, plane_bytes);
        hipLaunchKernelGGL(k_discard_line, dim3(h0), dim3(DISCARD_THREADS), 0, g_stream0, (const float *) c->bias0.get(), (const int32_t *) c->vs.get(), w0, thr, level,
                           depth, res + discard_result_off(0));
        g_discard_launches[0]++;
        HIPCK(hipGetLastError());
    }
    if (ranked) {
        ProfScope ps("discard_cross", g_stream0, plane_bytes);
        hipLaunchKernelGGL(k_discard_rank, dim3(h0), dim3(DISCARD_THREADS), 0, g_stream0, (const float *) c->bias0.get(), (const int32_t *) c->vs.get(), w0, w, thr, level,
                           depth, partial, res + discard_result_off(1));
        g_discard_launches[2]++;
        HIPCK(hipGetLastError());
        hipLaunchKernelGGL(k_discard_fold, dim3(discard_col_blocks(w)), dim3(DISCARD_THREADS), 0, g_stream0, (const int *) partial, w, 1, res + discard_result_off(1));
        g_discard_launches[3]++;
        HIPCK(hipGetLastError());
    } else if (cross) {
        ProfScope ps("discard_cross", g_stream0, plane_bytes + 8.0 * discard_partial_elems(w0, h0));
        hipLaunchKernelGGL(k_discard_cross, dim3(discard_col_blocks(w0), discard_row_tiles(h0)), dim3(DISCARD_THREADS), 0, g_stream0, (const float *) c->bias0.get(),
                           (const int32_t *) c->vs.get(), w0, h0, thr, level, depth, partial, res + discard_result_off(1));
        g_discard_launches[1]++;
        HIPCK(hipGetLastError());
        hipLaunchKernelGGL(k_discard_fold, dim3(discard_col_blocks(w0)), dim3(DISCARD_THREADS), 0, g_stream0, (const int *) partial, w0, discard_row_tiles(h0),
                           res + discard_result_off(1));
        g_discard_launches[3]++;
        HIPCK(hipGetLastError());
    }
    const int first = line ? 0 : 1, count = line && cross ? 2 : 1;
    if ((rc = d2h_staged(out + discard_result_off(first), res + discard_result_off(first), (size_t) count * DISCARD_WORDS * sizeof(int)))) return rc;
    tmp.done();
    return 0;
}

struct __attribute__((visibility("hidden"))) LqrHipForward {
    struct Planes {
        DevBuf<float> in, p;
        DevBuf<uint16_t> pos;
        DevBuf<int8_t> choice;
        DevBuf<int32_t> seam, map;
    };
    std::vector<Planes> img;
    std::vector<FwdJob> jobs;
    DevBuf<FwdJob> d_jobs;
    hipEvent_t slice_end[2] = {nullptr, nullptr};
    int slices = 0, next_seam = 0;
    int n = 0, L = 0, H = 0, depth = 0, orientation = 0, pxt = 0;
    size_t lds = 0;
    ~LqrHipForward()
    {
        if (g_stream0) (void) hipStreamSynchronize(g_stream0);
        for (hipEvent_t e : slice_end)
            if (e) (void) hipEventDestroy(e);
        (void) hipGetLastError();
    }
};
static std::atomic<unsigned long long> g_forward_launches{0};
extern "C" unsigned long long lqrhip_forward_launches(int reset)
{
    return reset ? g_forward_launches.exchange(0, std::memory_order_relaxed) : g_forward_launches.load(std::memory_order_relaxed);
}
static FwdJob forward_job(const LqrHipCarver *c, const LqrHipForward::Planes &pl, int32_t *map)
{
    return FwdJob{c->rgb0, c->bias0, pl.in, pl.p, pl.pos, pl.choice, pl.seam, map};
}
static int forward_launch_init(const LqrHipCarver *c0, const FwdJob *d_jobs, int n, int L, int H, int strided, int luma, int w_start, int orientation,
                               std::atomic<unsigned long long> &launches = g_forward_launches)
{
    DeepRead rd = deep_read(c0);
    rd.luma = luma != 0;
    const dim3 grid(tiles_of(L, 256), H, (unsigned) n);
#define CASE(D) if (c0->depth == D) hipLaunchKernelGGL(k_fwd_init<D>, grid, dim3(256), 0, g_stream0, d_jobs, L, H, c0->w0, strided, rd, w_start, orientation); else
    K_FWD_INIT_FORMS(CASE) return no_form("k_fwd_init");
#undef CASE
    launches.fetch_add(1, std::memory_order_relaxed);
    HIPCK(hipGetLastError());
    return 0;
}
extern "C" int lqrhip_forward_begin(LqrHipCarver *const *cs, int n, int depth, int orientation, int transposed, int luma, int w_start,
                                    void *const *device_maps, LqrHipForward **out)
{
    if (out) *out = nullptr;
    if (!cs || !out || n < 1 || n > LQRHIP_FORWARD_MAX_LINES || (orientation != 0 && orientation != 1) || w_start < 1) { g_err = "forward map: arguments"; return LQRHIP_EARG; }
    const LqrHipCarver *c0 = cs[0];
    for (int i = 0; i < n; i++) {
        const LqrHipCarver *c = cs[i];
        if (!c || c->root || c->w0 != c0->w0 || c->h0 != c0->h0 || c->ch != c0->ch || c->depth != c0->depth || c->mode != c0->mode ||
            c->alpha != c0->alpha || c->black != c0->black || (device_maps && !device_maps[i])) {
            g_err = "forward map: root carvers of one shape and pixel kind, a map for each";
            return LQRHIP_EARG;
        }
    }
    const int strided = (transposed != 0) != (orientation != 0);
    const int L = strided ? c0->h0 : c0->w0, H = strided ? c0->w0 : c0->h0;
    if (depth < 1 || depth >= L || L > FWD_THREADS * FWD_MAX_PXT || L > LQRHIP_MAX_FRAME_WIDTH || H > LQRHIP_FORWARD_MAX_LINES) {
        g_err = "forward map: 0 < depth < line length <= " + std::to_string(LQRHIP_MAX_FRAME_WIDTH) + ", at most " + std::to_string(LQRHIP_FORWARD_MAX_LINES) + " lines";
        return LQRHIP_EARG;
    }
    int rc;
    for (int i = 0; i < n; i++)
        if ((rc = batch_sync_of(cs[i]))) return rc;
    std::unique_ptr<LqrHipForward> f(new LqrHipForward());
    f->n = n; f->L = L; f->H = H; f->depth = depth; f->orientation = orientation;
    f->pxt = L <= FWD_THREADS ? 1 : L <= 2 * FWD_THREADS ? 2 : L <= 4 * FWD_THREADS ? 4 : L <= 8 * FWD_THREADS ? 8 : 16;
    f->lds = fwd_lds(L);
    const size_t px = (size_t) L * H;
    f->img.resize(n);
    for (int i = 0; i < n; i++) {
        LqrHipForward::Planes &pl = f->img[i];
        if ((rc = pl.in.alloc(px, "&fwd_in")) || (cs[i]->bias0 && (rc = pl.p.alloc(px, "&fwd_p"))) || (rc = pl.pos.alloc(px, "&fwd_pos")) ||
            (rc = pl.choice.alloc(px, "&fwd_choice")) || (rc = pl.seam.alloc((size_t) H, "&fwd_seam")) ||
            (!device_maps && (rc = pl.map.alloc(px, "&fwd_map"))))
            return rc;
        f->jobs.push_back(forward_job(cs[i], pl, device_maps ? (int32_t *) device_maps[i] : pl.map.get()));
    }
    if ((rc = f->d_jobs.alloc((size_t) n, "&fwd_jobs"))) return rc;
    for (hipEvent_t &e : f->slice_end) HIPCK(hipEventCreateWithFlags(&e, hipEventDisableTiming));
    if (lds_needs_attr(f->lds)) {
#define CASE(P) if (f->pxt == P) HIPCK(hipFuncSetAttribute((const void *) k_fwd_seam<P>, hipFuncAttributeMaxDynamicSharedMemorySize, (int) f->lds)); else
        K_FWD_SEAM_FORMS(CASE) return no_form("k_fwd_seam");
#undef CASE
    }
    HIPCK(hipMemcpyAsync(f->d_jobs, f->jobs.data(), (size_t) n * sizeof(FwdJob), hipMemcpyHostToDevice, g_stream0));
    if ((rc = forward_launch_init(c0, f->d_jobs, n, L, H, strided, luma, w_start, orientation))) return rc;
    *out = f.release();
    return 0;
}
extern "C" int lqrhip_forward_seams(LqrHipForward *f, int first_seam, int n_seams)
{
    if (!f || first_seam != f->next_seam || n_seams < 1 || first_seam + n_seams > f->depth) { g_err = "forward map: seams out of order or range"; return LQRHIP_EARG; }
    for (int s = first_seam; s < first_seam + n_seams; s++) {
        const int wc = f->L - s;
#define CASE(P) if (f->pxt == P) hipLaunchKernelGGL(k_fwd_seam<P>, dim3((unsigned) f->n), dim3(FWD_THREADS), f->lds, g_stream0, (const FwdJob *) f->d_jobs.get(), wc, f->L, f->H); else
        K_FWD_SEAM_FORMS(CASE) return no_form("k_fwd_seam");
#undef CASE
        hipLaunchKernelGGL(k_fwd_remove, dim3((unsigned) f->H, (unsigned) f->n), dim3(FWD_REMOVE_THREADS), 0, g_stream0, (const FwdJob *) f->d_jobs.get(), wc, f->L,
                           f->H, s + 1, f->orientation);
        g_forward_launches.fetch_add(2, std::memory_order_relaxed);
        HIPCK(hipGetLastError());
    }
    f->next_seam = first_seam + n_seams;
    HIPCK(hipEventRecord(f->slice_end[f->slices & 1], g_stream0));
    if (f->slices > 0) HIPCK(hipEventSynchronize(f->slice_end[(f->slices - 1) & 1]));
    f->slices++;
    return 0;
}
extern "C" int lqrhip_forward_finish(LqrHipForward *f)
{
    if (!f || f->next_seam != f->depth) { g_err = "forward map: the build is not complete"; return LQRHIP_EARG; }
    HIPCK(hipStreamSynchronize(g_stream0));
    return check_dev_error();
}
extern "C" const int *lqrhip_forward_map(const LqrHipForward *f, int i)
{
    return (f && i >= 0 && i < f->n) ? (const int *) f->jobs[i].map : nullptr;
}
extern "C" int lqrhip_forward_read_map(LqrHipForward *f, int i, int *out)
{
    if (!f || i < 0 || i >= f->n || !out) return LQRHIP_EARG;
    return d2h_staged(out, f->jobs[i].map, (size_t) f->L * f->H * sizeof(int32_t));
}
extern "C" void lqrhip_forward_release(LqrHipForward *f) { delete f; }
extern "C" int lqrhip_forward_intensity(LqrHipCarver *c, int orientation, int transposed, int luma, float *out)
{
    if (!c || c->root || !out || (orientation != 0 && orientation != 1)) return LQRHIP_EARG;
    int rc = batch_sync_of(c);
    if (rc) return rc;
    const int strided = (transposed != 0) != (orientation != 0);
    const int L = strided ? c->h0 : c->w0, H = strided ? c->w0 : c->h0;
    if (L > LQRHIP_MAX_FRAME_WIDTH || H > LQRHIP_FORWARD_MAX_LINES) return LQRHIP_EARG;
    const size_t px = (size_t) L * H;
    Scratch tmp(g_stream0);
    float *in = tmp.get<float>(px, "&fwd_in", rc);
    uint16_t *pos = rc ? nullptr : tmp.get<uint16_t>(px, "&fwd_pos", rc);
    int32_t *map = rc ? nullptr : tmp.get<int32_t>(px, "&fwd_map", rc);
    FwdJob *d_job = rc ? nullptr : tmp.get<FwdJob>(1, "&fwd_jobs", rc);
    if (rc) return rc;
    const FwdJob job{c->rgb0, nullptr, in, nullptr, pos, nullptr, nullptr, map};
    HIPCK(hipMemcpyAsync(d_job, &job, sizeof job, hipMemcpyHostToDevice, g_stream0));
    HIPCK(hipStreamSynchronize(g_stream0));
    if ((rc = forward_launch_init(c, d_job, 1, L, H, strided, luma, 1, orientation))) return rc;
    if ((rc = d2h_staged(out, in, px * sizeof(float)))) return rc;
    tmp.done();
    return 0;
}

struct __attribute__((visibility("hidden"))) LqrHipStatic {
    Scratch tmp{g_stream0};
    std::vector<StaticFrame> frames;
    StaticFrame *d_frames = nullptr;
    float *s = nullptr, *t = nullptr, *ip = nullptr, *e = nullptr;
    int n = 0, W = 0, H = 0, transposed = 0, orientation = 0, nrg = 0, depth = 0, next = 0;
    bool packed = false;
    float alpha = 0.0f;
    DeepRead rd{};
};
extern "C" int lqrhip_static_begin(LqrHipCarver *const *cs, int n, int orientation, int transposed, int nrg_func, float alpha, void *device_energy,
                                   LqrHipStatic **out)
{
    if (out) *out = nullptr;
    if (!cs || !out || n < 1 || n > LQRHIP_STATIC_MAX_FRAMES || (orientation != 0 && orientation != 1) || !(alpha >= 0.0f && alpha <= 1.0f)) {
        g_err = "static energy: arguments";
        return LQRHIP_EARG;
    }
    const LqrHipCarver *c0 = cs[0];
    for (int i = 0; i < n; i++) {
        const LqrHipCarver *c = cs[i];
        if (!c || c->root || c->w0 != c0->w0 || c->h0 != c0->h0 || c->ch != c0->ch || c->depth != c0->depth || c->mode != c0->mode ||
            c->alpha != c0->alpha || c->black != c0->black) {
            g_err = "static energy: root carvers of one shape and pixel kind";
            return LQRHIP_EARG;
        }
    }
    int rc;
    for (int i = 0; i < n; i++)
        if ((rc = batch_sync_of(cs[i]))) return rc;
    std::unique_ptr<LqrHipStatic> st(new LqrHipStatic());
    st->n = n; st->transposed = transposed != 0; st->orientation = orientation; st->alpha = alpha;
    st->W = transposed ? c0->h0 : c0->w0; st->H = transposed ? c0->w0 : c0->h0;
    const int nrg = nrg_index(nrg_func);
    st->nrg = plane_nrg(true, nrg);
    st->rd = deep_read(c0);
    st->rd.luma = nrg >= 3 && nrg <= 5;
    st->depth = c0->depth;
    st->packed = !reads_value(c0);
    const size_t px = (size_t) st->W * st->H;
    st->d_frames = st->tmp.get<StaticFrame>((size_t) n, "&static_frames", rc);
    if (rc) return rc;
    if (n > STATIC_GROUP) {
        if (!(st->s = st->tmp.get<float>(px, "&static_s", rc))) return rc;
        if (!(st->t = st->tmp.get<float>(px, "&static_t", rc))) return rc;
        if (!(st->ip = st->tmp.get<float>(px, "&static_i", rc))) return rc;
    }
    st->e = (float *) device_energy;
    if (!st->e && !(st->e = st->tmp.get<float>(px, "&static_e", rc))) return rc;
    for (int i = 0; i < n; i++) st->frames.push_back(StaticFrame{cs[i]->rgb0, cs[i]->bias0});
    HIPCK(hipMemcpyAsync(st->d_frames, st->frames.data(), (size_t) n * sizeof(StaticFrame), hipMemcpyHostToDevice, g_stream0));
    *out = st.release();
    return 0;
}
extern "C" int lqrhip_static_groups(const LqrHipStatic *st) { return st ? tiles_of(st->n, STATIC_GROUP) : 0; }
extern "C" int lqrhip_static_fold(LqrHipStatic *st)
{
    if (!st || st->next >= st->n) { g_err = "static energy: no frames left to fold"; return LQRHIP_EARG; }
    const int first = st->next, count = std::min(STATIC_GROUP, st->n - first);
    const bool last = first + count == st->n;
    const dim3 grid(tiles_of(st->W, STATIC_TILE), tiles_of(st->H, STATIC_TILE));
#define CASE(N, D, P) if (st->nrg == N && st->depth == D && st->packed == P) \
        hipLaunchKernelGGL((k_static_fold<N, D, P>), grid, dim3(STATIC_THREADS), 0, g_stream0, (const StaticFrame *) st->d_frames + first, count, first, st->W, st->H, \
                           st->transposed, st->orientation, st->rd, st->alpha, st->s, st->t, st->ip, last ? st->e : (float *) nullptr); else
    K_STATIC_FOLD_FORMS(CASE) return no_form("k_static_fold");
#undef CASE
    CENSUS(LQRHIP_CENSUS_STATIC_FOLD);
    HIPCK(hipGetLastError());
    st->next = first + count;
    return 0;
}
extern "C" int lqrhip_static_finish(LqrHipStatic *st, float *host_energy)
{
    if (!st || st->next != st->n) { g_err = "static energy: the fold is not complete"; return LQRHIP_EARG; }
    HIPCK(hipStreamSynchronize(g_stream0));
    int rc = check_dev_error();
    if (rc) return rc;
    if (host_energy && (rc = d2h_staged(host_energy, st->e, (size_t) st->W * st->H * sizeof(float)))) return rc;
    st->tmp.done();
    return 0;
}
extern "C" const float *lqrhip_static_energy(const LqrHipStatic *st) { return st ? st->e : nullptr; }
extern "C" void lqrhip_static_release(LqrHipStatic *st) { delete st; }

struct __attribute__((visibility("hidden"))) LqrHipClipFwd {
    Scratch tmp{g_stream0};
    std::vector<FwdJob> jobs;
    FwdJob *d_jobs = nullptr;
    float *in = nullptr, *cost = nullptr, *pm = nullptr;
    uint16_t *pos = nullptr;
    int8_t *choice = nullptr;
    int32_t *seam = nullptr, *map = nullptr;
    hipEvent_t slice_end[2] = {nullptr, nullptr};
    hipEvent_t fold_ends[2] = {nullptr, nullptr};
    int slices = 0, next_seam = 0;
    int n = 0, L = 0, H = 0, depth = 0, orientation = 0, pxt = 0;
    size_t lds = 0;
    ~LqrHipClipFwd()
    {
        if (g_stream0) (void) hipStreamSynchronize(g_stream0);
        tmp.done();
        for (hipEvent_t e : {slice_end[0], slice_end[1], fold_ends[0], fold_ends[1]})
            if (e) (void) hipEventDestroy(e);
        (void) hipGetLastError();
    }
};
static std::atomic<unsigned long long> g_clipfwd_launches{0};
extern "C" unsigned long long lqrhip_clipfwd_launches(int reset)
{
    return reset ? g_clipfwd_launches.exchange(0, std::memory_order_relaxed) : g_clipfwd_launches.load(std::memory_order_relaxed);
}
static std::atomic<double> g_clipfwd_fold_ms{0.0};
extern "C" double lqrhip_clipfwd_fold_ms(void) { return g_clipfwd_fold_ms.load(std::memory_order_relaxed); }
extern "C" int lqrhip_clipfwd_begin(LqrHipCarver *const *cs, int n, int depth, int orientation, int transposed, int luma, int w_start, float temporal,
                                    void *device_map, LqrHipClipFwd **out)
{
    if (out) *out = nullptr;
    if (!cs || !out || n < 1 || n > LQRHIP_FORWARD_MAX_LINES || (orientation != 0 && orientation != 1) || w_start < 1 ||
        !(temporal >= 0.0f && temporal <= 3.402823466e38f)) {
        g_err = "clip forward map: arguments";
        return LQRHIP_EARG;
    }
    const LqrHipCarver *c0 = cs[0];
    for (int i = 0; i < n; i++) {
        const LqrHipCarver *c = cs[i];
        if (!c || c->root || c->w0 != c0->w0 || c->h0 != c0->h0 || c->ch != c0->ch || c->depth != c0->depth || c->mode != c0->mode ||
            c->alpha != c0->alpha || c->black != c0->black || !c->bias0 != !c0->bias0) {
            g_err = "clip forward map: root carvers of one shape and pixel kind";
            return LQRHIP_EARG;
        }
    }
    const int strided = (transposed != 0) != (orientation != 0);
    const int L = strided ? c0->h0 : c0->w0, H = strided ? c0->w0 : c0->h0;
    if (depth < 1 || depth >= L || L > FWD_THREADS * FWD_MAX_PXT || L > LQRHIP_MAX_FRAME_WIDTH || H > LQRHIP_FORWARD_MAX_LINES) {
        g_err = "clip forward map: 0 < depth < line length <= " + std::to_string(LQRHIP_MAX_FRAME_WIDTH) + ", at most " + std::to_string(LQRHIP_FORWARD_MAX_LINES) + " lines";
        return LQRHIP_EARG;
    }
    int rc;
    for (int i = 0; i < n; i++)
        if ((rc = batch_sync_of(cs[i]))) return rc;
    std::unique_ptr<LqrHipClipFwd> f(new LqrHipClipFwd());
    f->n = n; f->L = L; f->H = H; f->depth = depth; f->orientation = orientation;
    f->pxt = L <= FWD_THREADS ? 1 : L <= 2 * FWD_THREADS ? 2 : L <= 4 * FWD_THREADS ? 4 : L <= 8 * FWD_THREADS ? 8 : 16;
    f->lds = fwd_lds(L);
    const size_t px = (size_t) L * H;
    if (!(f->in = f->tmp.get<float>(clip_intensity_elems(n, px), "&clip_in", rc))) return rc;
    if (!(f->cost = f->tmp.get<float>(clip_cost_elems(px), "&clip_cost", rc))) return rc;
    if (c0->bias0 && !(f->pm = f->tmp.get<float>(px, "&clip_pm", rc))) return rc;
    if (!(f->pos = f->tmp.get<uint16_t>(px, "&clip_pos", rc))) return rc;
    if (!(f->choice = f->tmp.get<int8_t>(px, "&clip_choice", rc))) return rc;
    if (!(f->seam = f->tmp.get<int32_t>((size_t) H, "&clip_seam", rc))) return rc;
    f->map = (int32_t *) device_map;
    if (!f->map && !(f->map = f->tmp.get<int32_t>(px, "&clip_map", rc))) return rc;
    if (!(f->d_jobs = f->tmp.get<FwdJob>((size_t) n, "&clip_jobs", rc))) return rc;
    for (int i = 0; i < n; i++)
        f->jobs.push_back(FwdJob{cs[i]->rgb0, cs[i]->bias0, f->in + clip_frame_off(i, px), nullptr, f->pos, nullptr, nullptr, f->map});
    for (hipEvent_t &e : f->slice_end) HIPCK(hipEventCreateWithFlags(&e, hipEventDisableTiming));
    for (hipEvent_t &e : f->fold_ends) HIPCK(hipEventCreate(&e));
    if (lds_needs_attr(f->lds)) {
#define CASE(P) if (f->pxt == P) HIPCK(hipFuncSetAttribute((const void *) k_clip_seam<P>, hipFuncAttributeMaxDynamicSharedMemorySize, (int) f->lds)); else
        K_CLIP_SEAM_FORMS(CASE) return no_form("k_clip_seam");
#undef CASE
    }
    HIPCK(hipMemcpyAsync(f->d_jobs, f->jobs.data(), (size_t) n * sizeof(FwdJob), hipMemcpyHostToDevice, g_stream0));
    if ((rc = forward_launch_init(c0, f->d_jobs, n, L, H, strided, luma, w_start, orientation, g_clipfwd_launches))) return rc;
    const dim3 grid(tiles_of(L, CLIPFWD_FOLD_THREADS), H);
    HIPCK(hipEventRecord(f->fold_ends[0], g_stream0));
    for (int g = 0; g < clip_fold_groups(n, CLIPFWD_GROUP); g++) {
        const int first = g * CLIPFWD_GROUP, count = std::min(CLIPFWD_GROUP, n - first);
        hipLaunchKernelGGL(k_clip_fold, grid, dim3(CLIPFWD_FOLD_THREADS), 0, g_stream0, (const FwdJob *) f->d_jobs, (const float *) f->in, first, count,
                           first + count == n ? 1 : 0, L, H, c0->w0, strided, w_start, temporal, f->cost, f->pm);
        g_clipfwd_launches.fetch_add(1, std::memory_order_relaxed);
        HIPCK(hipGetLastError());
    }
    HIPCK(hipEventRecord(f->fold_ends[1], g_stream0));
    *out = f.release();
    return 0;
}
extern "C" int lqrhip_clipfwd_seams(LqrHipClipFwd *f, int first_seam, int n_seams)
{
    if (!f || first_seam != f->next_seam || n_seams < 1 || first_seam + n_seams > f->depth) { g_err = "clip forward map: seams out of order or range"; return LQRHIP_EARG; }
    for (int s = first_seam; s < first_seam + n_seams; s++) {
        const int wc = f->L - s;
#define CASE(P) if (f->pxt == P) hipLaunchKernelGGL(k_clip_seam<P>, dim3(1), dim3(FWD_THREADS), f->lds, g_stream0, (const float *) f->cost, f->choice, f->seam, wc, f->L, f->H); else
        K_CLIP_SEAM_FORMS(CASE) return no_form("k_clip_seam");
#undef CASE
        hipLaunchKernelGGL(k_clip_remove, dim3((unsigned) f->H), dim3(FWD_REMOVE_THREADS), 0, g_stream0, f->cost, f->pos, (const int32_t *) f->seam, f->map, wc, f->L, f->H,
                           s + 1, f->orientation);
        g_clipfwd_launches.fetch_add(2, std::memory_order_relaxed);
        if (s + 1 < f->depth) {
            hipLaunchKernelGGL(k_clip_refresh, dim3((unsigned) f->H), dim3(CLIPFWD_REFRESH_THREADS), 0, g_stream0, (const float *) f->in, f->n, f->cost,
                               (const uint16_t *) f->pos, (const int32_t *) f->seam, wc - 1, f->L, f->H);
            g_clipfwd_launches.fetch_add(1, std::memory_order_relaxed);
        }
        HIPCK(hipGetLastError());
    }
    f->next_seam = first_seam + n_seams;
    HIPCK(hipEventRecord(f->slice_end[f->slices & 1], g_stream0));
    if (f->slices > 0) HIPCK(hipEventSynchronize(f->slice_end[(f->slices - 1) & 1]));
    f->slices++;
    return 0;
}
extern "C" int lqrhip_clipfwd_finish(LqrHipClipFwd *f)
{
    if (!f || f->next_seam != f->depth) { g_err = "clip forward map: the build is not complete"; return LQRHIP_EARG; }
    HIPCK(hipStreamSynchronize(g_stream0));
    float ms = 0.0f;
    if (hipEventElapsedTime(&ms, f->fold_ends[0], f->fold_ends[1]) == hipSuccess) g_clipfwd_fold_ms.store(ms, std::memory_order_relaxed);
    (void) hipGetLastError();
    return check_dev_error();
}
extern "C" const int *lqrhip_clipfwd_map(const LqrHipClipFwd *f) { return f ? (const int *) f->map : nullptr; }
extern "C" int lqrhip_clipfwd_read_map(LqrHipClipFwd *f, int *out)
{
    if (!f || !out) return LQRHIP_EARG;
    return d2h_staged(out, f->map, (size_t) f->L * f->H * sizeof(int32_t));
}
extern "C" void lqrhip_clipfwd_release(LqrHipClipFwd *f) { delete f; }

extern "C" int lqrhip_mask_line_max(const unsigned char *mask, int channels, int width, int height, int a0, int b0, int n_lines,
                                    int line_len, int direction)
{
    if (lqrhip_init() < 0) return LQRHIP_EHIP;
    if (n_lines <= 0 || line_len <= 0) return 0;
    int rc, result = 0;
    size_t bytes = (size_t) width * height * channels;
    Scratch tmp(g_stream0);
    uint8_t *d = tmp.get<uint8_t>(bytes, "&d", rc);
    if (rc) return rc;
    int *dout = tmp.get<int>(1, "&dout", rc);
    if (rc) return rc;
    HIPCK(hipMemcpyAsync(d, mask, bytes, hipMemcpyHostToDevice, g_stream0));
    HIPCK(hipMemsetAsync(dout, 0, sizeof(int), g_stream0));
    hipLaunchKernelGGL(k_mask_line_max, dim3(n_lines), dim3(256), 0, g_stream0, d, channels, width, a0, b0, line_len, direction, dout);
    HIPCK(hipGetLastError());
    HIPCK(hipMemcpyAsync(&result, dout, sizeof(int), hipMemcpyDeviceToHost, g_stream0));
    HIPCK(hipStreamSynchronize(g_stream0));
    tmp.done();
    return result;
}

extern "C" void lqrhip_pool_trim(void)
{
    (void) hipDeviceSynchronize();
    g_cache.trim();
    unpark_all();
}

extern "C" int lqrhip_device_sync(void)
{
    HIPCK(hipDeviceSynchronize());
    return check_dev_error();
}

extern "C" int lqrhip_read_vmap(LqrHipCarver *c, int w0, int h0, int w, int level, int depth, int *out)
{
    int rc = batch_sync_of(c);
    if (rc) return rc;
    size_t n = (size_t) w * h0;
    Scratch tmp(g_stream0);
    int32_t *d = tmp.get<int32_t>(n, "&d", rc);
    if (rc) return rc;
    hipLaunchKernelGGL(k_compact<false>, dim3(h0), dim3(256), 0, g_stream0, (const uint8_t *) nullptr, vs_of(c), (const float *) nullptr,
                       (const float *) nullptr, (uint8_t *) nullptr, (float *) nullptr, (float *) nullptr, d, w0, w, c->ch, level,
                       depth);
    HIPCK(hipGetLastError());
    if ((rc = d2h_staged(out, d, n * sizeof(int32_t)))) return rc;
    tmp.done();
    return 0;
}

extern "C" int lqrhip_read_seam_flags(LqrHipCarver *c, int *org, int *org_prev, int *side)
{
    int rc = batch_sync_of(c);
    if (rc) return rc;
    if (!c->wk.flags) return LQRHIP_EARG;
    int32_t fl[FLAG_COUNT];
    HIPCK(hipMemcpy(fl, c->wk.flags, sizeof fl, hipMemcpyDeviceToHost));
    *org = fl[FLAG_ORG]; *org_prev = fl[FLAG_ORG_PREV]; *side = fl[FLAG_SIDE];
    return 0;
}
extern "C" int lqrhip_read_working(LqrHipCarver *c, int w, int h, float *en, float *m, int *least_dx)
{
    int rc = batch_sync_of(c);
    if (rc) return rc;
    if (!c->wk.pix) return LQRHIP_EARG;
    int32_t fl[FLAG_COUNT];
    HIPCK(hipMemcpy(fl, c->wk.flags, sizeof fl, hipMemcpyDeviceToHost));
    const int org = fl[FLAG_ORG];
    size_t n = (size_t) c->stride * h;
    std::vector<float> t(n);
    std::vector<int8_t> tl(n);
    if (en) {
        HIPCK(hipMemcpy(t.data(), c->wk.en, n * sizeof(float), hipMemcpyDeviceToHost));
        for (int y = 0; y < h; y++) memcpy(en + (size_t) y * w, t.data() + (size_t) y * c->stride + org, (size_t) w * sizeof(float));
    }
    if (m) {
        HIPCK(hipMemcpy(t.data(), c->wk.m, n * sizeof(float), hipMemcpyDeviceToHost));
        for (int y = 0; y < h; y++) memcpy(m + (size_t) y * w, t.data() + (size_t) y * c->stride + org, (size_t) w * sizeof(float));
    }
    if (least_dx) {
        HIPCK(hipMemcpy(tl.data(), c->wk.least, n, hipMemcpyDeviceToHost));
        for (int y = 0; y < h; y++)
            for (int x = 0; x < w; x++) least_dx[(size_t) y * w + x] = y == 0 ? 0 : (int) tl[(size_t) y * c->stride + org + x];
    }
    return 0;
}

__global__ __launch_bounds__(256) void k_copy16(const u32x4 *__restrict__ src, u32x4 *__restrict__ dst, size_t n16);
static int reset_planes(LqrHipCarver *c, int w, int h)
{
    int rc = batch_sync_of(c);
    if (rc) return rc;
    const size_t n = (size_t) w * h;
    c->rgb0.reset(); c->vs.reset(); c->bias0.reset(); c->rig0.reset();
    if (c->wk.bias || c->wk.rig) { free_working(c); c->stride = 0; c->wk_h = 0; }
    c->w0 = w; c->h0 = h;
    drop_catchup(c);
    if ((rc = c->rgb0.alloc(n * px_bytes(c), "&c->rgb0")) || (rc = c->vs.alloc(n, "&c->vs"))) return rc;
    return 0;
}
extern "C" int lqrhip_carver_reset(LqrHipCarver *c, const void *device_rgb, int w, int h)
{
    if (!c || c->root || !c->aux.empty() || w < 1 || h < 1) return LQRHIP_EARG;
    int rc = reset_planes(c, w, h);
    if (rc) return rc;
    const size_t n = (size_t) w * h;
    {
        const size_t bytes = n * px_bytes(c), n16 = bytes / 16;
        if (n16 && !(((uintptr_t) device_rgb | (uintptr_t) c->rgb0.get()) & 15)) {
            hipLaunchKernelGGL(k_copy16, dim3((unsigned) blocks_of(n16, 256)), dim3(256), 0, g_stream0, (const u32x4 *) device_rgb, (u32x4 *) c->rgb0.get(), n16);
            HIPCK(hipGetLastError());
            if (bytes & 15) HIPCK(hipMemcpyAsync(c->rgb0 + n16 * 16, (const uint8_t *) device_rgb + n16 * 16, bytes & 15, hipMemcpyDeviceToDevice, g_stream0));
        } else {
            HIPCK(hipMemcpyAsync(c->rgb0, device_rgb, bytes, hipMemcpyDeviceToDevice, g_stream0));
        }
    }
    HIPCK(hipMemsetAsync(c->vs, 0, n * sizeof(int32_t), g_stream0));
    if (c->batch) c->batch->dirty = true;
    if (c->active && (rc = ensure_working(c, w, h))) return rc;
    return 0;
}

enum { RESET_JOBS = 16 };
struct ResetJob { const uint8_t *src; uint8_t *dst; uint8_t *vs; size_t bytes; };
struct ResetJobs { ResetJob j[RESET_JOBS]; };
__global__ __launch_bounds__(256) void k_reset_jobs(const ResetJobs jobs, const size_t vs_bytes);
static int g_reset_batch_count = 0;
extern "C" int lqrhip_carver_reset_batch_count(void) { return g_reset_batch_count; }
extern "C" int lqrhip_carver_reset_batch(LqrHipCarver **cs, const void *const *device_rgb, int n, int w, int h)
{
    g_reset_batch_count = 0;
    if (!cs || !device_rgb || n < 1 || w < 1 || h < 1) return LQRHIP_EARG;
    for (int i = 0; i < n; i++)
        if (!cs[i] || cs[i]->root || !cs[i]->aux.empty() || !device_rgb[i]) return LQRHIP_EARG;
    const size_t npx = (size_t) w * h, vs_bytes = npx * sizeof(int32_t);
    ResetJobs jobs = {};
    int nj = 0;
    size_t most = vs_bytes;
    auto flush = [&]() -> int {
        if (!nj) return 0;
        const unsigned blocks = (unsigned) std::min<size_t>(blocks_of(most / 16, 256) + 1, 4096);
        hipLaunchKernelGGL(k_reset_jobs, dim3(blocks, (unsigned) nj), dim3(256), 0, g_stream0, jobs, vs_bytes);
        nj = 0; most = vs_bytes;
        HIPCK(hipGetLastError());
        return 0;
    };
    for (int i = 0; i < n; i++) {
        LqrHipCarver *c = cs[i];
        g_reset_batch_count = i;
        int rc = reset_planes(c, w, h);
        if (rc) { (void) flush(); return rc; }
        const size_t bytes = npx * px_bytes(c);
        if (!(((uintptr_t) device_rgb[i] | (uintptr_t) c->rgb0.get() | (uintptr_t) c->vs.get()) & 15)) {
            jobs.j[nj++] = ResetJob{(const uint8_t *) device_rgb[i], c->rgb0.get(), (uint8_t *) c->vs.get(), bytes};
            most = std::max(most, bytes);
            g_fixed_stats[1]++;
        } else {
            g_fixed_stats[2]++;
            hipError_t e = hipMemcpyAsync(c->rgb0, device_rgb[i], bytes, hipMemcpyDeviceToDevice, g_stream0);
            if (e == hipSuccess) e = hipMemsetAsync(c->vs, 0, vs_bytes, g_stream0);
            if (e != hipSuccess) { (void) flush(); HIPCK(e); }
        }
        if (c->batch) c->batch->dirty = true;
        if (c->active && (rc = ensure_working(c, w, h))) { (void) flush(); return rc; }
        if (nj == RESET_JOBS && (rc = flush())) return rc;
    }
    int rc = flush();
    if (rc) return rc;
    g_reset_batch_count = n;
    return 0;
}

extern "C" int lqrhip_reset_sync(void)
{
    if (g_stream0) HIPCK(hipStreamSynchronize(g_stream0));
    return 0;
}

extern "C" int lqrhip_mem_info(unsigned long long *free_bytes, unsigned long long *total_bytes, unsigned long long *cached_bytes)
{
// ... 99 lines not shown
```

gimp-lqr-plugin_amd/host/lqr_carver.c:

```c
#ifdef LQRHIP_TIMING
#define _POSIX_C_SOURCE 199309L
#endif
#include <stdlib.h>
#include <string.h>
#include <stdio.h>
#include <math.h>

#include "../../include/lqr.h"
#include "../../include/lqr_coldepth.h"
#include "../../include/lqr_imagetype.h"
#include "../../include/lqr_masks.h"
#include "../../include/lqr_energy.h"
#include "../../include/lqr_vmap.h"
#include "../../include/lqr_control.h"
#include "../../include/lqr_sizes.h"
#include "../../include_ext/lqr_forward.h"
#include "../../include_ext/lqr_static.h"
#include "../../include_ext/lqr_clipforward.h"
#include "../../include_ext/lqr_remove.h"
#include "../../include/lqr_hip.h"
#include "lqr_mask_queue.h"
#include "lqr_sched.h"
#include "lqr_state.h"

// ... 700 lines not shown
    rc = lqr_maskq_append(q, (size_t) r->geo.w0 * r->geo.h0, index, v);
    if (rc == LQR_MASKQ_FULL) {
        LQR_CATCH(mask_queue_flush_one(r, is_rig));
        rc = lqr_maskq_append(q, (size_t) r->geo.w0 * r->geo.h0, index, v);
    }
    return rc == LQR_MASKQ_OK ? LQR_OK : rc == LQR_MASKQ_NOMEM ? LQR_NOMEM : LQR_ERROR;
}
LqrRetVal lqr_carver_bias_add_xy(LqrCarver *r, gdouble bias, gint x, gint y)
{
    if (bias == 0) return LQR_OK;
    return mask_add_xy(r, 0, bias, x, y);
}
LqrRetVal lqr_carver_rigmask_add_xy(LqrCarver *r, gdouble rigidity, gint x, gint y) { return mask_add_xy(r, 1, rigidity, x, y); }

static void mask_clear(LqrCarver *r, int is_rig)
{
    lqr_maskq_reset(&r->mq[is_rig]);
    (void) hip_ret(lqrhip_mask_clear(r->dev, is_rig));
    if (is_rig) r->has_rigmask = 0; else r->has_bias = 0;
    r->wk_valid = 0;
}
void lqr_carver_bias_clear(LqrCarver *r) { mask_clear(r, 0); }
void lqr_carver_rigmask_clear(LqrCarver *r) { mask_clear(r, 1); }

static LqrRetVal mask_read(LqrCarver *r, int is_rig, gfloat *out)
{
    LQR_CATCH(mask_queue_flush(r));
    if (lqr_geom_needs_flatten(&r->geo)) return LQR_ERROR;
    HIP_CATCH(lqrhip_read_mask_plane(r->dev, is_rig, r->geo.transposed, out));
    return LQR_OK;
}
LqrRetVal lqrx_carver_get_bias(LqrCarver *r, gfloat *out) { return mask_read(r, 0, out); }
LqrRetVal lqrx_carver_get_rigmask(LqrCarver *r, gfloat *out) { return mask_read(r, 1, out); }

static LqrRetVal take_debug_snapshot(LqrCarver *r)
{
    size_t n = (size_t) r->geo.w * r->geo.h;
    free(r->dbg_en); free(r->dbg_m); free(r->dbg_least);
    r->dbg_w = r->geo.w; r->dbg_h = r->geo.h;
    r->dbg_en = (float *) malloc(n * sizeof(float));
    r->dbg_m = (float *) malloc(n * sizeof(float));
    r->dbg_least = (int *) malloc(n * sizeof(int));
    if (!r->dbg_en || !r->dbg_m || !r->dbg_least) return LQR_NOMEM;
    HIP_CATCH(lqrhip_read_working(r->dev, r->geo.w, r->geo.h, r->dbg_en, r->dbg_m, r->dbg_least));
    HIP_CATCH(lqrhip_read_seam_flags(r->dev, &r->dbg_org, &r->dbg_org_prev, &r->dbg_side));
    return LQR_OK;
}

static LqrRetVal group_build_vsmap(Group *g, const LqrSession *s, int *reported)
{
    LqrCarver *r0 = g->r[0];
    LqrHipDpParams p;
    int l, i;
    dp_params(r0, &p);
    HIP_ALL(g, lqrhip_seam_log_reserve(B, s->n_seams, r0->geo.h));

    for (l = s->max_level; l < s->depth; l++) {
        const int lr_pick = r0->leftright;
        LqrSeam seam;
        lqr_session_seam(s, l, &seam);
        if (seam.report && r0->progress && r0->progress->update) {
            HIP_ALL(g, lqrhip_batch_sync(B));
            if (l > *reported) {
                r0->progress->update(seam.fraction);
                *reported = l;
            }
            CANCEL_POINT(g);
        }
        CANCEL_POINT(g);
        if (seam.full)
            for (i = 0; i < g->n; i++) g->r[i]->leftright ^= 1;
        HIP_ALL(g, lqrhip_seam_step(B, &p, seam.w_before, r0->geo.h, l - s->max_level, lr_pick, seam.full, r0->leftright));
        for (i = 0; i < g->n; i++) { g->r[i]->geo.level++; g->r[i]->geo.w--; }
    }

    if (g_debug_snapshot)
        for (i = 0; i < g->n; i++) LQR_CATCH(take_debug_snapshot(g->r[i]));

    T_BEGIN(T_TAIL);
    HIP_ALL(g, lqrhip_session_check(B, r0->geo.h, s->wc0, s->n_seams, r0->delta_x));
    HIP_ALL(g, lqrhip_batch_sync(B));
    HIP_ALL(g, lqrhip_vs_commit(B, r0->geo.w0, r0->geo.h0, s->wc0, s->n_seams, s->first_level, s->finish));
    for (i = 0; i < g->n; i++) (void) lqr_state_phase(&g->r[i]->state, LQR_STATE_INFLATING);
    HIP_ALL(g, lqrhip_inflate(B, r0->geo.w0, r0->geo.h0, s->depth - 1, s->max_level));
    HIP_ALL(g, lqrhip_planes_commit(B));
    T_END(T_TAIL);
    FOR_TREE(g, i, r, {
        lqr_geom_session_done(&r->geo, s->depth, s->n_seams);
        ro_invalidate(r);
    });
    return LQR_OK;
}

static LqrRetVal session_run(Group *g, const LqrSession *s, int redo, int *reported)
{
    LqrCarver *r0 = g->r[0];
    LqrHipDpParams p;
    int i;
    LQR_CATCH(group_phase(g, LQR_STATE_RESIZING));
    for (i = 0; i < g->n; i++) set_width_one(g->r[i], s->wc0);
    dp_params(r0, &p);
    if (!r0->wk_valid || redo) {
        const int from_visible = (r0->geo.max_level != 1 || r0->geo.w0 != r0->geo.w_start);
        if (from_visible) HIP_ALL(g, lqrhip_wk_init(B, 1));
        else HIP_ALL(g, lqrhip_wk_init_emap(B, &p, r0->geo.w, r0->geo.h));
        for (i = 0; i < g->n; i++) g->r[i]->wk_valid = 1;
        if (from_visible) HIP_ALL(g, lqrhip_emap_build(B, &p, r0->geo.w, r0->geo.h));
    } else
        HIP_ALL(g, lqrhip_emap_build(B, &p, r0->geo.w, r0->geo.h));
    HIP_ALL(g, lqrhip_mmap_build(B, &p, r0->geo.w, r0->geo.h, r0->leftright));
    return group_build_vsmap(g, s, reported);
}

static LqrRetVal group_build_maps(Group *g, int depth)
{
    LqrCarver *r0 = g->r[0];
    LqrSession s;
    LqrRetVal ret;
    int i, k, reported = -1, *snap;
    if (depth <= r0->geo.max_level) return LQR_OK;
    if (!r0->active || r0->root) return LQR_ERROR;
    lqr_session_begin(&s, r0->geo.max_level, depth, r0->geo.w_start - r0->geo.max_level + 1, r0->lr_switch_frequency, r0->session_rescale_current,
                      r0->session_rescale_total, r0->session_update_step);
    snap = (int *) malloc((size_t) g->n * 3 * sizeof *snap);
    if (!snap) return LQR_NOMEM;
    for (i = 0; i < g->n; i++) { snap[3 * i] = g->r[i]->geo.w; snap[3 * i + 1] = g->r[i]->geo.level; snap[3 * i + 2] = g->r[i]->leftright; }
    g_last_rc = 0;
    ret = session_run(g, &s, 0, &reported);
    for (k = 0; k < 2 && ret != LQR_OK; k++) {
        const int fault = (ret == LQR_ERROR && g_last_rc == LQRHIP_EFAULT);
        const int cancelled = (ret == LQR_USRCANCEL);
        if (fault || cancelled || g_last_rc == LQRHIP_ENOMEM)
            for (i = 0; i < g->nb; i++) (void) lqrhip_session_rollback(g->b[i], r0->geo.w0, r0->geo.h0, s.first_level, s.finish);
        for (i = 0; i < g->n; i++) {
            LqrCarver *c = g->r[i];
            c->geo.w = snap[3 * i]; c->geo.level = snap[3 * i + 1]; c->leftright = snap[3 * i + 2];
            c->wk_valid = 0;
            ro_invalidate(c);
        }
        if (!fault || !lqrhip_get_recovery() || k == 1) break;
        fprintf(stderr, "liblqr-hip: the session is carved again on the kernels without spin waits\n");
        for (i = 0; i < g->nb; i++) lqrhip_batch_set_safe(g->b[i], 1);
        g_last_rc = 0;
        ret = session_run(g, &s, 1, &reported);
        for (i = 0; i < g->nb; i++) lqrhip_batch_set_safe(g->b[i], 0);
    }
    free(snap);
    return ret;
}

LqrVMap *lqr_vmap_dump(LqrCarver *r)
{
    LqrVMap *v;
    int w = r->geo.w_start, h = r->geo.h, depth = r->geo.w0 - r->geo.w_start, x, y;
    int *frame, *buffer;
    frame = (int *) malloc((size_t) w * h * sizeof(int));
    v = (LqrVMap *) calloc(1, sizeof *v);
    if (!frame || !v) { free(frame); free(v); return NULL; }
    if (lqrhip_read_vmap(r->dev, r->geo.w0, r->geo.h0, w, r->geo.w0 - w + 1, depth, frame) != 0) {
        fprintf(stderr, "liblqr-hip: vmap read-back failed: %s\n", lqrhip_last_error());
        free(frame); free(v);
        return NULL;
    }
    if (r->geo.transposed) {
        buffer = (int *) malloc((size_t) w * h * sizeof(int));
        if (!buffer) { free(frame); free(v); return NULL; }
        for (y = 0; y < h; y++)
            for (x = 0; x < w; x++) buffer[(size_t) x * h + y] = frame[(size_t) y * w + x];
// ... 491 lines not shown
}

LqrVMap *lqrx_clip_forward_map(LqrCarver **frames, gint n, gint depth, gint orientation, gfloat temporal)
{
    LqrHipClipFwd *f;
    LqrVMap *v = NULL;
    gint *buffer;
    int L, width, height;
    if (clipfwd_check(frames, n, 1, depth, orientation, temporal, "lqrx_clip_forward_map", &L) != LQR_OK) return NULL;
    if (roots_enter(frames, n, LQR_STATE_RESIZING) != LQR_OK) return NULL;
    width = lqr_carver_get_width(frames[0]); height = lqr_carver_get_height(frames[0]);
    buffer = (gint *) malloc((size_t) width * height * sizeof *buffer);
    if (buffer && clipfwd_build_entered(frames, n, depth, orientation, temporal, L, NULL, &f) == LQR_OK) {
        if (hip_ret(lqrhip_clipfwd_read_map(f, buffer)) == LQR_OK) v = lqr_vmap_new(buffer, width, height, depth, orientation);
        lqrhip_clipfwd_release(f);
    }
    if (!v) free(buffer);
    roots_leave(frames, n);
    return v;
}

LqrRetVal lqrx_clip_load_forward(LqrCarver **frames, gint n, gint depth, gint orientation, gfloat temporal)
{
    LqrHipClipFwd *f;
    LqrRetVal ret;
    int L;
    LQR_CATCH(clipfwd_check(frames, n, 1, depth, orientation, temporal, "lqrx_clip_load_forward", &L));
    LQR_CATCH(roots_enter(frames, n, LQR_STATE_RESIZING));
    ret = clipfwd_build_entered(frames, n, depth, orientation, temporal, L, NULL, &f);
    if (ret == LQR_OK) {
        ret = group_vmap_load_entered(frames, n, lqrhip_clipfwd_map(f), 1, lqr_carver_get_width(frames[0]), lqr_carver_get_height(frames[0]), depth, orientation);
        lqrhip_clipfwd_release(f);
    }
    roots_leave(frames, n);
    return ret;
}

LqrRetVal lqrx_clip_resize_forward(LqrCarver **frames, gint n, gint w1, gint h1, gfloat temporal)
{
    int w, h, dir, k;
    LQR_CATCH(clipfwd_check(frames, n, 0, 0, 0, temporal, "lqrx_clip_resize_forward", &k));
    w = lqr_carver_get_width(frames[0]); h = lqr_carver_get_height(frames[0]);
    if (w1 < 1 || h1 < 1 || abs(w1 - w) >= w || abs(h1 - h) >= h || (w1 != w && w > LQRHIP_MAX_FRAME_WIDTH) || (h1 != h && h > LQRHIP_MAX_FRAME_WIDTH) ||
        (w1 != w && MAXI(h, h1) > LQRHIP_FORWARD_MAX_LINES) || (h1 != h && MAXI(w, w1) > LQRHIP_FORWARD_MAX_LINES)) {
        fprintf(stderr, "liblqr-hip: lqrx_clip_resize_forward refused: %d x %d to %d x %d (a change below the line length, lines of at most %d, "
                "at most %d of them)\n", w, h, w1, h1, LQRHIP_MAX_FRAME_WIDTH, LQRHIP_FORWARD_MAX_LINES);
        return LQR_ERROR;
    }
    LQR_CATCH(roots_enter(frames, n, LQR_STATE_RESIZING));
    roots_leave(frames, n);
    for (k = 0; k < 2; k++) {
        dir = (frames[0]->resize_order == LQR_RES_ORDER_HOR) ? k : 1 - k;
        w = lqr_carver_get_width(frames[0]); h = lqr_carver_get_height(frames[0]);
        if ((dir ? h1 - h : w1 - w) == 0) continue;
        LQR_CATCH(lqrx_clip_load_forward(frames, n, abs(dir ? h1 - h : w1 - w), dir, temporal));
        LQR_CATCH(lqrx_carver_resize_batch(frames, n, dir ? w : w1, dir ? h1 : h));
    }
    return LQR_OK;
}

static LqrRetVal group_resize_dir(Group *g, int w1, int want_transposed)
{
    LqrCarver *r = g->r[0];
    LqrWalk walk;
    LqrWalkStep s;
    int i;
    const gchar *init_msg = want_transposed ? r->progress->init_height_message : r->progress->init_width_message;
    const gchar *end_msg = want_transposed ? r->progress->end_height_message : r->progress->end_width_message;

    lqr_walk_begin(&walk, &r->geo, r->enl_step, w1, want_transposed);
    if (walk.total) CANCEL_POINT(g);
    for (i = 0; i < g->n; i++) {
        LqrCarver *c = g->r[i];
        c->session_rescale_total = walk.total;
        c->session_rescale_current = 0;
        c->session_update_step = lqr_sched_update_step(walk.total, c->progress->update_step);
    }
    if (walk.total && r->progress->init) r->progress->init(init_msg);

    while (lqr_walk_next(&walk, &s)) {
        CANCEL_POINT(g);
        if (s.transpose) LQR_CATCH(group_transpose(g));
        LQR_CATCH(group_build_maps(g, s.depth));
        for (i = 0; i < g->n; i++) {
            set_width_tree(g->r[i], s.new_w);
            g->r[i]->session_rescale_current = walk.total - (s.gamma > 0 ? s.gamma : -s.gamma);
            if (g->r[i]->dump_vmaps) LQR_CATCH(lqr_vmap_internal_dump(g->r[i]));
        }
        if (s.flatten) LQR_CATCH(group_flatten(g));
    }
    if (walk.total && r->progress->end) {
        HIP_ALL(g, lqrhip_batch_sync(B));
        r->progress->end(end_msg);
    }
    return LQR_OK;
}

static int same_config(const LqrCarver *a, const LqrCarver *b)
{
    LqrCarverList *la = a->attached, *lb = b->attached;
    if (a->geo.w0 != b->geo.w0 || a->geo.h0 != b->geo.h0 || a->geo.w != b->geo.w || a->geo.h != b->geo.h || a->geo.w_start != b->geo.w_start ||
        a->geo.h_start != b->geo.h_start || a->geo.level != b->geo.level || a->geo.max_level != b->geo.max_level || a->channels != b->channels ||
        a->geo.transposed != b->geo.transposed || a->active != b->active || a->delta_x != b->delta_x || a->rigidity != b->rigidity ||
        a->has_bias != b->has_bias || a->has_rigmask != b->has_rigmask || a->nrg_func != b->nrg_func ||
        a->leftright != b->leftright || a->lr_switch_frequency != b->lr_switch_frequency || a->enl_step != b->enl_step ||
        a->resize_order != b->resize_order || a->wk_valid != b->wk_valid || a->col_depth != b->col_depth ||
        a->image_type != b->image_type || a->alpha_channel != b->alpha_channel || a->black_channel != b->black_channel)
        return 0;
    for (; la && lb; la = la->next, lb = lb->next)
        if (la->current->channels != lb->current->channels || la->current->col_depth != lb->current->col_depth) return 0;
    return !la && !lb;
}

static int frame_refused(const LqrCarver *r, int w1, int want_transposed)
{
    return lqr_walk_frame_refused(&r->geo, r->enl_step, w1, want_transposed, LQRHIP_MAX_FRAME_WIDTH);
}
static int inactive_refused(const LqrCarver *r, int w1, int want_transposed)
{
    return !r->active && lqr_walk_needs_maps(&r->geo, r->enl_step, w1, want_transposed);
}

static LqrRetVal group_resize_entered(LqrCarver **rs, int n, int w1, int h1);
static LqrRetVal group_resize(LqrCarver **rs, int n, int w1, int h1)
{
    LqrRetVal ret;
    int i;
    if (w1 < 1 || h1 < 1) return LQR_ERROR;
    for (i = 0; i < n; i++)
        if (rs[i]->root || !rs[i]->progress) return LQR_ERROR;
    LQR_CATCH(roots_enter(rs, n, LQR_STATE_RESIZING));
    ret = group_resize_entered(rs, n, w1, h1);
    roots_leave(rs, n);
    return ret;
}
static LqrRetVal group_resize_entered(LqrCarver **rs, int n, int w1, int h1)
{
    Group g;
    LqrRetVal ret = LQR_OK;
    int i;
    for (i = 0; i < n; i++) LQR_CATCH(mask_queue_flush(rs[i]));
    for (i = 0; i < n; i++)
        if (frame_refused(rs[i], w1, 0) || frame_refused(rs[i], h1, 1)) {
            fprintf(stderr, "liblqr-hip: resize refused: a frame wider than %d px in the direction being carved is not supported\n",
                    LQRHIP_MAX_FRAME_WIDTH);
            return LQR_ERROR;
        }
    for (i = 0; i < n; i++)
        if (inactive_refused(rs[i], w1, 0) || inactive_refused(rs[i], h1, 1)) return LQR_ERROR;
    {
        T_BEGIN(T_OPEN);
        LQR_CATCH(group_open(&g, rs, n));
        T_END(T_OPEN);
    }
    if (rs[0]->resize_order == LQR_RES_ORDER_HOR) {
        if ((ret = group_resize_dir(&g, w1, 0)) == LQR_OK) ret = group_resize_dir(&g, h1, 1);
    } else {
        if ((ret = group_resize_dir(&g, h1, 1)) == LQR_OK) ret = group_resize_dir(&g, w1, 0);
    }
    if (ret == LQR_OK) {
        int k;
        for (k = 0; k < g.nb; k++) { LqrRetVal rk = hip_ret(lqrhip_batch_sync(g.b[k])); if (ret == LQR_OK) ret = rk; }
    }
    if (ret != LQR_OK) { int k; for (k = 0; k < g.nb; k++) lqrhip_batch_abort(g.b[k]); }
    FOR_TREE(&g, i, r, ro_invalidate(r));
    {
// ... 401 lines not shown
```

include/lqr_hip.h:

```cpp
#ifndef LQR_HIP_H
#define LQR_HIP_H

#include <stddef.h>

#ifdef __cplusplus
extern "C" {
#endif

#define LQRHIP_OK 0
#define LQRHIP_ENOMEM (-2)
#define LQRHIP_EHIP (-1)
#define LQRHIP_EARG (-3)
#define LQRHIP_EFAULT (-4)
#define LQRHIP_EMAP (-5)
#define LQRHIP_MAX_DELTA 16
#define LQRHIP_MAX_CHANNELS 64
#define LQRHIP_MAX_FRAME_WIDTH 16384

typedef struct LqrHipCarver LqrHipCarver;
typedef struct LqrHipBatch LqrHipBatch;

typedef struct LqrHipDpParams {
    int delta_x;
    int use_rigidity;
    float rigidity_map[2 * LQRHIP_MAX_DELTA + 1];
    int nrg_func;
    int nrg_radius;
    int w_start;
} LqrHipDpParams;

int lqrhip_init(void);
const char *lqrhip_last_error(void);

LqrHipCarver *lqrhip_carver_create(const unsigned char *rgb, int w, int h, int channels);
LqrHipCarver *lqrhip_carver_create_ext(const void *rgb, int w, int h, int channels, int depth);
int lqrhip_carver_set_read_luma(LqrHipCarver *c, int luma);
int lqrhip_carver_set_read(LqrHipCarver *c, int image_type, int alpha, int black);
void lqrhip_carver_destroy(LqrHipCarver *c);
int lqrhip_carver_reset(LqrHipCarver *c, const void *device_rgb, int w, int h);
int lqrhip_carver_reset_batch(LqrHipCarver **cs, const void *const *device_rgb, int n, int w, int h);
int lqrhip_carver_reset_batch_count(void);
int lqrhip_reset_sync(void);
int lqrhip_carver_attach(LqrHipCarver *root, LqrHipCarver *aux);
int lqrhip_carver_activate(LqrHipCarver *c);

int lqrhip_mask_add(LqrHipCarver *c, const unsigned char *mask, int channels, int width, int height,
                    int x_off, int y_off, int transposed, int is_rigmask, int bias_factor);

int lqrhip_mask_add_f(LqrHipCarver *c, const void *mask, int depth, int on_device, int width, int height, int x_off, int y_off,
                      int transposed, int is_rigmask, int bias_factor);
int lqrhip_mask_plane_ensure(LqrHipCarver *c, int is_rigmask);
int lqrhip_mask_scatter(LqrHipCarver *c, int is_rigmask, const int *index, const double *value, const size_t *start, int buckets);
int lqrhip_mask_clear(LqrHipCarver *c, int is_rigmask);
int lqrhip_read_mask_plane(LqrHipCarver *c, int is_rigmask, int transposed, float *out);
unsigned long long lqrhip_debug_mask_flushes(void);

int lqrhip_sub_batches(int n);
int lqrhip_general_batch_limit(int w);
int lqrhip_general_batch_limit_delta(int w, int delta_x);
void lqrhip_set_sub_batches(int n);
LqrHipBatch *lqrhip_batch_create(LqrHipCarver **carvers, int n);
void lqrhip_batch_set_shared(LqrHipBatch *b, int shared);
void lqrhip_batch_destroy(LqrHipBatch *b);
int lqrhip_batch_sync(LqrHipBatch *b);
void lqrhip_batch_abort(LqrHipBatch *b);
void *lqrhip_batch_stream(LqrHipBatch *b);

int lqrhip_wk_init(LqrHipBatch *b, int from_visible);
int lqrhip_emap_build(LqrHipBatch *b, const LqrHipDpParams *p, int w, int h);
int lqrhip_wk_init_emap(LqrHipBatch *b, const LqrHipDpParams *p, int w, int h);
int lqrhip_energy_out(LqrHipBatch *b, int w, int h, int transposed, int form, int depth, int image_type, void *out, int on_device);
int lqrhip_mmap_build(LqrHipBatch *b, const LqrHipDpParams *p, int w, int h, int leftright);
int lqrhip_seam_step(LqrHipBatch *b, const LqrHipDpParams *p, int w, int h, int log_index,
                     int leftright_pick, int full_rebuild, int leftright_next);
int lqrhip_seam_log_reserve(LqrHipBatch *b, int n_seams, int h);
int lqrhip_vs_commit(LqrHipBatch *b, int w0, int h0, int wc0, int n_seams, int first_level, int finish);
int lqrhip_session_check(LqrHipBatch *b, int h, int wc0, int n_seams, int delta_x);
void lqrhip_set_selfcheck(int on);
void lqrhip_set_recovery(int on);
int lqrhip_get_recovery(void);
int lqrhip_session_rollback(LqrHipBatch *b, int w0, int h0, int first_level, int finish);
void lqrhip_batch_set_safe(LqrHipBatch *b, int safe);
void lqrhip_set_no_spin(int on);
int lqrhip_get_no_spin(void);
int lqrhip_fault_stats(unsigned long long *out8, int reset);
void lqrhip_debug_inject(int kind, int at_step, int times);
void lqrhip_debug_fail_alloc(int nth);
unsigned long long lqrhip_debug_pool_live(void);
void lqrhip_debug_fixedcost(unsigned long long out4[4], int reset);
int lqrhip_inflate(LqrHipBatch *b, int w0, int h0, int l, int max_level);
typedef struct LqrHipVMap LqrHipVMap;
int lqrhip_vmap_stage(const int *map, int on_device, int width, int height, int depth, int orientation, LqrHipVMap **out);
int lqrhip_vmap_load(LqrHipBatch *b, const LqrHipVMap *m);
void lqrhip_vmap_release(LqrHipVMap *m);
int lqrhip_flatten(LqrHipBatch *b, int w0, int h0, int w, int level);
int lqrhip_transpose(LqrHipBatch *b, int w, int h);
int lqrhip_planes_commit(LqrHipBatch *b);
int lqrhip_inflate_commit(LqrHipBatch *b);

int lqrhip_read_visible(LqrHipCarver *c, int w0, int h0, int w, int level, unsigned char *out);
int lqrhip_mask_line_max(const unsigned char *mask, int channels, int width, int height, int a0, int b0, int n_lines, int line_len,
                         int direction);
int lqrhip_read_visible_device(LqrHipCarver *c, int w0, int h0, int w, int level, void *device_out);
int lqrhip_read_sizes(LqrHipCarver *c, int w0, int h0, int transposed, const int *levels, int n, void *const *outs, int on_device);
#define LQRHIP_DISCARD_LINE 1
#define LQRHIP_DISCARD_CROSS 2
int lqrhip_discard_scan(LqrHipCarver *c, int w0, int h0, int w, int level, int depth, float strength, int which, int *out);
void lqrhip_discard_launches(unsigned long long out4[4], int reset);
#define LQRHIP_FORWARD_MAX_LINES 65535
typedef struct LqrHipForward LqrHipForward;
int lqrhip_forward_begin(LqrHipCarver *const *cs, int n, int depth, int orientation, int transposed, int luma, int w_start,
                         void *const *device_maps, LqrHipForward **out);
int lqrhip_forward_seams(LqrHipForward *f, int first_seam, int n_seams);
int lqrhip_forward_finish(LqrHipForward *f);
const int *lqrhip_forward_map(const LqrHipForward *f, int i);
int lqrhip_forward_read_map(LqrHipForward *f, int i, int *out);
void lqrhip_forward_release(LqrHipForward *f);
unsigned long long lqrhip_forward_launches(int reset);
int lqrhip_forward_intensity(LqrHipCarver *c, int orientation, int transposed, int luma, float *out);
int lqrhip_read_forward_intensity(const void *carver, int orientation, float *out);
#define LQRHIP_STATIC_MAX_FRAMES 65535
typedef struct LqrHipStatic LqrHipStatic;
int lqrhip_static_begin(LqrHipCarver *const *cs, int n, int orientation, int transposed, int nrg_func, float alpha, void *device_energy,
                        LqrHipStatic **out);
int lqrhip_static_groups(const LqrHipStatic *st);
int lqrhip_static_fold(LqrHipStatic *st);
int lqrhip_static_finish(LqrHipStatic *st, float *host_energy);
const float *lqrhip_static_energy(const LqrHipStatic *st);
void lqrhip_static_release(LqrHipStatic *st);
typedef struct LqrHipClipFwd LqrHipClipFwd;
int lqrhip_clipfwd_begin(LqrHipCarver *const *cs, int n, int depth, int orientation, int transposed, int luma, int w_start, float temporal,
                         void *device_map, LqrHipClipFwd **out);
int lqrhip_clipfwd_seams(LqrHipClipFwd *f, int first_seam, int n_seams);
int lqrhip_clipfwd_finish(LqrHipClipFwd *f);
const int *lqrhip_clipfwd_map(const LqrHipClipFwd *f);
int lqrhip_clipfwd_read_map(LqrHipClipFwd *f, int *out);
void lqrhip_clipfwd_release(LqrHipClipFwd *f);
unsigned long long lqrhip_clipfwd_launches(int reset);
double lqrhip_clipfwd_fold_ms(void);
int lqrhip_device_sync(void);
int lqrhip_mem_info(unsigned long long *free_bytes, unsigned long long *total_bytes, unsigned long long *cached_bytes);
int lqrhip_copy_bandwidth(unsigned long long bytes, int iters, double *gbps);
int lqrhip_vmap_to_rgba(const int *vmap, int w, int h, int depth, const double col_start[3], const double col_end[3],
                        unsigned char *out_rgba);
void lqrhip_pool_trim(void);
int lqrhip_read_vmap(LqrHipCarver *c, int w0, int h0, int w, int level, int depth, int *out);
int lqrhip_read_working(LqrHipCarver *c, int w, int h, float *en, float *m, int *least_dx);
int lqrhip_read_seam_flags(LqrHipCarver *c, int *org, int *org_prev, int *side);
int lqrhip_debug_seam_flags(const void *carver, int *org, int *org_prev, int *side);

void lqrhip_prof_enable(int on);
void lqrhip_set_update_mode(int mode);
void lqrhip_set_sweep_threads(int n);
void lqrhip_set_carve_fused(int max_images);
void lqrhip_set_carve_beside(int mode);
unsigned long long lqrhip_carve_beside_launches(int reset);
void lqrhip_set_backtrack_beside(int mode);
unsigned long long lqrhip_backtrack_beside_launches(int reset);
void lqrhip_set_vpath_mode(int mode, int par_max);
void lqrhip_set_dp_persistent_limit(int workgroups);
void lqrhip_set_dp_persistent_px(int px);
void lqrhip_prof_reset(void);
int lqrhip_prof_get(const char *kernel, double *ms_total, long long *launches, double *bytes_total);
int lqrhip_prof_get_union(const char *kernel, double *ms_union);
int lqrhip_moved_bytes(unsigned long long *bytes, int reset);
void lqrhip_set_band_levels(int slots);
void lqrhip_set_levels_wg_slots(int slots);
void lqrhip_set_carve_line(int mode);
void lqrhip_set_levels_store(int mode);
unsigned long long lqrhip_levels_pair_launches(int reset);
int lqrhip_band_levels_stats(unsigned long long *out8, int reset);
enum {
    LQRHIP_CENSUS_VP_PARALLEL = 0,
// ... 31 lines not shown
```

Before: 623,700 Mseams*px/s.

## Defer inflate after seam sessions until a consumer needs the inflated layout

Adds a lazy-inflate mode in which the session tail records an owed inflate per carver rather than running the inflate kernels and plane commit right away. Each entry point either pays the debt, drops it, or translates levels so reads and flattening work directly on the un-inflated base layout. In a shrink-only run the inflate pass (a full-plane rewrite across all images, plus a sync) can then be skipped entirely, with a light census kernel kept as a self-check. The cost is a good deal of bookkeeping across many entry points, with a risk of stale or inconsistent state if some path misses the debt.

```diff
diff --git a/gimp-lqr-plugin_amd/csrc/k_oneoff.hip b/gimp-lqr-plugin_amd/csrc/k_oneoff.hip
--- a/gimp-lqr-plugin_amd/csrc/k_oneoff.hip
+++ b/gimp-lqr-plugin_amd/csrc/k_oneoff.hip
@@ -83,6 +83,28 @@
     if (dev_err && (twice || (tid == 0 && carry != n_levels))) dev_fail(dev_err, DEVERR_LEVELS);
 }
 
+__global__ __launch_bounds__(256) void k_levels_census(const DevCarver *cs, int w0, int first_level, int n_levels, int *dev_err)
+{
+    extern __shared__ unsigned s_seen[];
+    __shared__ int s_cnt;
+    const GCarver c = gview_phys(cs[blockIdx.y]);
+    const int tid = threadIdx.x;
+    for (int i = tid; i < (n_levels + 31) / 32; i += 256) s_seen[i] = 0u;
+    if (tid == 0) s_cnt = 0;
+    __syncthreads();
+    const gi32 *vrow = c.vs + (size_t) blockIdx.x * w0;
+    bool twice = false;
+    int cnt = 0;
+    for (int x = tid; x < w0; x += 256) {
+        const int k = vrow[x] - first_level;
+        if (k >= 0 && k < n_levels) { twice |= (atomicOr(&s_seen[k >> 5], 1u << (k & 31)) >> (k & 31)) & 1u; cnt++; }
+    }
+    for (int o = 32; o > 0; o >>= 1) cnt += __shfl_down(cnt, o);
+    if ((tid & 63) == 0) atomicAdd(&s_cnt, cnt);
+    __syncthreads();
+    if (twice || (tid == 0 && s_cnt != n_levels)) dev_fail(dev_err, DEVERR_LEVELS);
+}
+
 __global__ __launch_bounds__(256) void k_vmap_check(const int32_t *map, int len, int depth, int *dev_err)
 {
     extern __shared__ unsigned s_seen[];
diff --git a/gimp-lqr-plugin_amd/csrc/lqr_kernels.h b/gimp-lqr-plugin_amd/csrc/lqr_kernels.h
--- a/gimp-lqr-plugin_amd/csrc/lqr_kernels.h
+++ b/gimp-lqr-plugin_amd/csrc/lqr_kernels.h
@@ -71,6 +71,7 @@
 
 __global__ __launch_bounds__(256) void k_vs_commit(const DevCarver *cs, int w0, int h0, int wc0, int n_seams, int first_level, int finish);
 template <bool DEEP> __global__ __launch_bounds__(256) void k_inflate(const InflateDev *jobs, int w0, int w1, int l, int max_level, int *dev_err);
+__global__ __launch_bounds__(256) void k_levels_census(const DevCarver *cs, int w0, int first_level, int n_levels, int *dev_err);
 __global__ __launch_bounds__(256) void k_vmap_check(const int32_t *map, int len, int depth, int *dev_err);
 __global__ __launch_bounds__(256) void k_vmap_check_t(const int32_t *map, int32_t *out, int width, int height, int depth, int *dev_err);
 __global__ __launch_bounds__(256) void k_seam_check(const DevCarver *cs, int h, int wc0, int n_seams, int delta, int *dev_err);
diff --git a/gimp-lqr-plugin_amd/csrc/lqr_shim.hip b/gimp-lqr-plugin_amd/csrc/lqr_shim.hip
--- a/gimp-lqr-plugin_amd/csrc/lqr_shim.hip
+++ b/gimp-lqr-plugin_amd/csrc/lqr_shim.hip
@@ -3,6 +3,7 @@
 #include "lqr_own.h"
 #include "lqr_pool.h"
 #include "lqr_stage.h"
+#include "../host/lqr_owed.h"
 #include <atomic>
 #include <memory>
 #include <dirent.h>
@@ -52,6 +53,7 @@
     int log_cap = 0, log_h = 0;
     int frozen_epoch = 0;
     int owed_to = 0, owed_w = 0, owed_h = 0;
+    LqrOwed owed_inflate = {0, 0};
     LqrHipCarver *root = nullptr;
     std::vector<LqrHipCarver *> aux;
     LqrHipBatch *batch = nullptr;
@@ -434,6 +436,41 @@
     c->frozen_epoch = 0;
 }
 
+static int g_inflate_lazy = -1;
+static unsigned long long g_inflate_passes = 0;
+static inline LqrHipCarver *root_of(LqrHipCarver *c) { return c->root ? c->root : c; }
+static int pay_inflate(LqrHipCarver *const *roots, size_t n, hipStream_t s);
+static int owed_enter(LqrHipCarver *c, int entry, int level = 0, int first_level = 0, int *act = nullptr)
+{
+    LqrHipCarver *r = root_of(c);
+    const int a = lqr_owed_action(&r->owed_inflate, entry, level, first_level);
+    if (act) *act = a == LQR_OWED_TRANSLATE ? a : LQR_OWED_IGNORE;
+    if (a == LQR_OWED_DROP) r->owed_inflate = LqrOwed{0, 0};
+    if (a != LQR_OWED_PAY) return 0;
+    if (r->batch) HIPCK(hipStreamSynchronize(r->batch->stream));
+    return pay_inflate(&r, 1, g_stream0);
+}
+static int owed_enter_batch(LqrHipBatch *b, int entry, int level = 0, int first_level = 0, LqrOwed *translate = nullptr)
+{
+    size_t n_pay = 0, n_translate = 0;
+    bool alike = true;
+    const LqrHipCarver *t0 = nullptr;
+    for (auto *c : b->cs) {
+        const int a = lqr_owed_action(&c->owed_inflate, entry, level, first_level);
+        if (a == LQR_OWED_DROP) c->owed_inflate = LqrOwed{0, 0};
+        else if (a == LQR_OWED_PAY) n_pay++;
+        else if (a == LQR_OWED_TRANSLATE) {
+            if (!t0) t0 = c;
+            alike &= c->owed_inflate.l == t0->owed_inflate.l && c->owed_inflate.max_level == t0->owed_inflate.max_level && c->w0 == t0->w0 && c->h0 == t0->h0;
+            n_translate++;
+        }
+    }
+    if (translate) *translate = LqrOwed{0, 0};
+    if (n_translate && translate && alike && n_translate == b->cs.size()) { *translate = t0->owed_inflate; return 0; }
+    if (!n_pay && !n_translate) return 0;
+    return pay_inflate(b->cs.data(), b->cs.size(), b->stream);
+}
+
 static void free_working(LqrHipCarver *c)
 {
     c->wk = WorkingPlanes();
@@ -456,6 +493,8 @@
 
 extern "C" int lqrhip_carver_attach(LqrHipCarver *root, LqrHipCarver *aux)
 {
+    int rc;
+    if ((rc = owed_enter(root, LQR_OWED_AT_ATTACH)) || (rc = owed_enter(aux, LQR_OWED_AT_ATTACH))) return rc;
     if (root->w0 != aux->w0 || root->h0 != aux->h0) return LQRHIP_EARG;
     aux->vs.reset();
     aux->root = root;
@@ -506,16 +545,19 @@
 
 extern "C" int lqrhip_carver_activate(LqrHipCarver *c)
 {
+    int rc = owed_enter(c, LQR_OWED_AT_ACTIVATE);
+    if (rc) return rc;
     c->active = 1;
     return ensure_working(c, c->w0, c->h0);
 }
 
 extern "C" int lqrhip_mask_plane_ensure(LqrHipCarver *c, int is_rigmask)
 {
+    int rc = owed_enter(c, LQR_OWED_AT_MASK_WRITE);
+    if (rc) return rc;
     DevBuf<float> &plane = is_rigmask ? c->rig0 : c->bias0;
     if (plane) return 0;
-    int rc = batch_sync_of(c);
-    if (rc) return rc;
+    if ((rc = batch_sync_of(c))) return rc;
     const size_t n = (size_t) c->w0 * c->h0;
     if ((rc = plane.alloc(n, "plane"))) return rc;
     hipError_t e = dzero(plane, n * sizeof(float));
@@ -621,7 +663,7 @@
 extern "C" int lqrhip_read_mask_plane(LqrHipCarver *c, int is_rigmask, int transposed, float *out)
 {
     int rc = batch_sync_of(c);
-    if (rc) return rc;
+    if (rc || (rc = owed_enter(c, LQR_OWED_AT_MASK_READ))) return rc;
     const size_t n = (size_t) c->w0 * c->h0;
     const float *plane = is_rigmask ? c->rig0 : c->bias0;
     if (!plane) { memset(out, 0, n * sizeof(float)); return 0; }
@@ -847,7 +889,9 @@
 extern "C" int lqrhip_wk_init(LqrHipBatch *b, int from_visible)
 {
     LqrHipCarver *c0 = b->cs[0];
-    int w = c0->w0, h = c0->h0, rc;
+    int rc;
+    if ((rc = owed_enter_batch(b, LQR_OWED_AT_WK_INIT))) return rc;
+    const int w = c0->w0, h = c0->h0;
     if ((rc = wk_init_prepare(b))) return rc;
     const dim3 grid(tiles_of(c0->stride, 256), h, (unsigned) b->cs.size()), grid_v(h, (unsigned) b->cs.size());
 #define LAUNCH_WK(FORM, arg) do { if (from_visible) hipLaunchKernelGGL(k_wk_init_visible<FORM>, grid_v, dim3(256), 0, b->stream, b->d_desc, w, h, c0->stride, arg); \
@@ -883,6 +927,7 @@
 {
     LqrHipCarver *c0 = b->cs[0];
     int rc;
+    if ((rc = owed_enter_batch(b, LQR_OWED_AT_WK_INIT))) return rc;
     if (reads_value(c0) || w != c0->w0 || h != c0->h0) return (rc = lqrhip_wk_init(b, 0)) ? rc : lqrhip_emap_build(b, p, w, h);
     if ((rc = wk_init_prepare(b))) return rc;
     const dim3 grid(tiles_of(tiles_of(c0->stride, 4), 256), h, (unsigned) b->cs.size());
@@ -1370,6 +1415,7 @@
 extern "C" int lqrhip_seam_log_reserve(LqrHipBatch *b, int n_seams, int h)
 {
     int rc;
+    if ((rc = owed_enter_batch(b, LQR_OWED_AT_SESSION))) return rc;
     if ((rc = pay_catchup(b))) return rc;
     for (auto *c : b->cs) if ((rc = ensure_log(c, n_seams, h))) return rc;
     return 0;
@@ -1378,6 +1424,7 @@
 extern "C" int lqrhip_vs_commit(LqrHipBatch *b, int w0, int h0, int wc0, int n_seams, int first_level, int finish)
 {
     int rc;
+    if ((rc = owed_enter_batch(b, LQR_OWED_AT_SESSION))) return rc;
     if ((rc = batch_upload(b))) return rc;
     size_t lds = vsc_lds(n_seams, wc0);
     if (lds > VSC_LDS_MAX) { g_err = "vs_commit: session too large for LDS"; return LQRHIP_EARG; }
@@ -1417,8 +1464,9 @@
     if (g_dev_err_host) *g_dev_err_host = 0;
     invalidate_all_batches();
     int rc;
+    (void) owed_enter_batch(b, LQR_OWED_AT_ROLLBACK, 0, first_level);
     if ((rc = batch_upload(b))) return rc;
-    const size_t n = (size_t) w0 * h0;
+    const size_t n = std::min((size_t) w0 * h0, (size_t) b->cs[0]->w0 * b->cs[0]->h0);
     hipLaunchKernelGGL(k_vs_rollback, dim3((unsigned) std::min<size_t>(blocks_of(n, 256), 4096), (unsigned) b->cs.size()), dim3(256), 0, b->stream, b->d_desc, n, first_level, finish ? w0 : 0);
     HIPCK(hipGetLastError());
     HIPCK(hipStreamSynchronize(b->stream));
@@ -1458,13 +1506,14 @@
     int kept() { keep = true; return 0; }
 };
 }
-static int inflate_stage(LqrHipBatch *b, int w0, int h0, int l, int max_level, const int32_t *levels)
+static int inflate_run(PlaneJobs &pj, LqrHipCarver *const *roots, size_t n, hipStream_t s, int w0, int h0, int l, int max_level, const int32_t *levels,
+                       int *dev_err)
 {
     int rc;
     const int w1 = w0 + l - max_level + 1;
-    Staging st(b, 0, w1, h0);
-    PlaneJobs &pj = st.jobs();
-    for (auto *c : b->cs) {
+    pj.new_vs.reserve(n);
+    for (size_t i = 0; i < n; i++) {
+        LqrHipCarver *c = roots[i];
         pj.new_vs.emplace_back();
         DevBuf<int32_t> &nvs = pj.new_vs.back();
         if ((rc = nvs.alloc((size_t) w1 * h0, "&nvs"))) return rc;
@@ -1473,18 +1522,80 @@
             if ((rc = pj.add(a, vs, nullptr, (size_t) w1 * h0))) return rc;
         if ((rc = pj.add(c, vs, nvs, (size_t) w1 * h0))) return rc;
     }
-    if ((rc = pj.stage(b->stream, false))) return rc;
+    if ((rc = pj.stage(s, false))) return rc;
     const size_t lds = inflate_lds(l, max_level);
     if (pj.n_narrow)
-        hipLaunchKernelGGL(k_inflate<false>, dim3(h0, (unsigned) pj.n_narrow), dim3(256), lds, b->stream, pj.d_dev.get(), w0, w1, l, max_level, g_selfcheck ? g_dev_err : (int *) nullptr);
+        hipLaunchKernelGGL(k_inflate<false>, dim3(h0, (unsigned) pj.n_narrow), dim3(256), lds, s, pj.d_dev.get(), w0, w1, l, max_level, dev_err);
     if (pj.n_wide())
-        hipLaunchKernelGGL(k_inflate<true>, dim3(h0, (unsigned) pj.n_wide()), dim3(256), lds, b->stream, pj.d_wide(), w0, w1, l, max_level, g_selfcheck ? g_dev_err : (int *) nullptr);
+        hipLaunchKernelGGL(k_inflate<true>, dim3(h0, (unsigned) pj.n_wide()), dim3(256), lds, s, pj.d_wide(), w0, w1, l, max_level, dev_err);
+    g_inflate_passes++;
+    HIPCK(hipGetLastError());
+    HIPCK(hipStreamSynchronize(s));
+    return 0;
+}
+static int inflate_stage(LqrHipBatch *b, int w0, int h0, int l, int max_level, const int32_t *levels)
+{
+    int rc;
+    if ((rc = owed_enter_batch(b, LQR_OWED_AT_INFLATE))) return rc;
+    Staging st(b, 0, w0 + l - max_level + 1, h0);
+    if ((rc = inflate_run(st.jobs(), b->cs.data(), b->cs.size(), b->stream, w0, h0, l, max_level, levels, g_selfcheck ? g_dev_err : (int *) nullptr))) return rc;
+    if ((rc = check_dev_error())) return rc;
+    return st.kept();
+}
+static int pay_inflate(LqrHipCarver *const *roots, size_t n, hipStream_t s)
+{
+    std::vector<LqrHipCarver *> todo;
+    for (size_t i = 0; i < n; i++)
+        if (lqr_owed_any(&roots[i]->owed_inflate)) todo.push_back(roots[i]);
+    if (todo.empty()) return 0;
+    if (g_stream0 && s != g_stream0) HIPCK(hipStreamSynchronize(g_stream0));
+    while (!todo.empty()) {
+        LqrHipCarver *c0 = todo.front();
+        const LqrOwed o = c0->owed_inflate;
+        std::vector<LqrHipCarver *> same, rest;
+        for (auto *c : todo)
+            (c->owed_inflate.l == o.l && c->owed_inflate.max_level == o.max_level && c->w0 == c0->w0 && c->h0 == c0->h0 ? same : rest).push_back(c);
+        PlaneJobs pj;
+        const int rc = inflate_run(pj, same.data(), same.size(), s, c0->w0, c0->h0, o.l, o.max_level, nullptr, nullptr);
+        if (rc) { lqr_stream_wait(s); return rc; }
+        const int w1 = c0->w0 + lqr_owed_seams(&o), h1 = c0->h0;
+        commit(pj);
+        for (auto &j : pj.jobs) { j.c->w0 = w1; j.c->h0 = h1; if (j.c->batch) j.c->batch->dirty = true; }
+        for (size_t i = 0; i < same.size(); i++) {
+            same[i]->vs = std::move(pj.new_vs[i]);
+            same[i]->owed_inflate = LqrOwed{0, 0};
+        }
+        todo.swap(rest);
+    }
+    return 0;
+}
+extern "C" int lqrhip_inflate(LqrHipBatch *b, int w0, int h0, int l, int max_level) { return inflate_stage(b, w0, h0, l, max_level, nullptr); }
+
+extern "C" void lqrhip_set_inflate_lazy(int mode) { g_inflate_lazy = mode == 0 ? 0 : mode > 0 ? 1 : -1; }
+extern "C" int lqrhip_get_inflate_lazy(void) { return g_inflate_lazy != 0; }
+extern "C" unsigned long long lqrhip_inflate_launches(int reset) { const unsigned long long n = g_inflate_passes; if (reset) g_inflate_passes = 0; return n; }
+extern "C" int lqrhip_levels_check(LqrHipBatch *b, int w0, int h0, int l, int max_level)
+{
+    int rc;
+    if ((rc = batch_upload(b))) return rc;
+    for (auto *c : b->cs)
+        if (c->w0 != w0 || c->h0 != h0 || !c->vs) { g_err = "levels check: the carver's base layout is not the session's"; return LQRHIP_EARG; }
+    if (g_selfcheck && l >= max_level)
+        hipLaunchKernelGGL(k_levels_census, dim3(h0, (unsigned) b->cs.size()), dim3(256), inflate_lds(l, max_level), b->stream, b->d_desc, w0, 2 * max_level - 1,
+                           l - max_level + 1, g_dev_err);
     HIPCK(hipGetLastError());
     HIPCK(hipStreamSynchronize(b->stream));
-    if ((rc = check_dev_error())) return rc;
-    return st.kept();
-}
-extern "C" int lqrhip_inflate(LqrHipBatch *b, int w0, int h0, int l, int max_level) { return inflate_stage(b, w0, h0, l, max_level, nullptr); }
+    return check_dev_error();
+}
+extern "C" int lqrhip_inflate_pay(LqrHipBatch *b) { return owed_enter_batch(b, LQR_OWED_AT_WIDTH); }
+extern "C" int lqrhip_inflate_owe(LqrHipBatch *b, int w0, int h0, int l, int max_level)
+{
+    if (l < max_level || max_level < 1) return LQRHIP_EARG;
+    for (auto *c : b->cs)
+        if (c->w0 != w0 || c->h0 != h0 || lqr_owed_any(&c->owed_inflate)) { g_err = "inflate: the carver's base layout is not the session's"; return LQRHIP_EARG; }
+    for (auto *c : b->cs) c->owed_inflate = LqrOwed{l, max_level};
+    return 0;
+}
 
 struct __attribute__((visibility("hidden"))) LqrHipVMap {
     DevBuf<int32_t> own;
@@ -1550,7 +1661,7 @@
     commit(pj);
     for (auto &j : pj.jobs) { j.c->w0 = pi->w1; j.c->h0 = pi->h1; }
     if (pi->kind != 0)
-        for (auto *c : b->cs) drop_catchup(c);
+        for (auto *c : b->cs) { drop_catchup(c); (void) owed_enter(c, LQR_OWED_AT_COMMIT_FLAT); }
     if (pi->kind != 2) {
         size_t i = 0;
         for (auto *c : b->cs) c->vs = std::move(pj.new_vs[i++]);
@@ -1564,6 +1675,9 @@
 extern "C" int lqrhip_flatten(LqrHipBatch *b, int w0, int h0, int w, int level)
 {
     int rc;
+    LqrOwed owed;
+    if ((rc = owed_enter_batch(b, LQR_OWED_AT_FLATTEN, level, 0, &owed))) return rc;
+    if (lqr_owed_any(&owed)) { w0 = b->cs[0]->w0; level = lqr_owed_level(&owed, level); }
     Staging st(b, 1, w, h0);
     PlaneJobs &pj = st.jobs();
     for (auto *c : b->cs) {
@@ -1588,6 +1702,7 @@
 extern "C" int lqrhip_transpose(LqrHipBatch *b, int w, int h)
 {
     int rc;
+    if ((rc = owed_enter_batch(b, LQR_OWED_AT_TRANSPOSE))) return rc;
     Staging st(b, 2, h, w);
     PlaneJobs &pj = st.jobs();
     for (auto *c : b->cs) {
@@ -1613,10 +1728,17 @@
     if (px_bytes(c) > 4) LAUNCH_RV(true); else LAUNCH_RV(false);
 #undef LAUNCH_RV
 }
+static int read_visible_enter(LqrHipCarver *c, int &w0, int &level)
+{
+    int act;
+    const int rc = owed_enter(c, LQR_OWED_AT_READ_VISIBLE, level, 0, &act);
+    if (!rc && act == LQR_OWED_TRANSLATE) { w0 = c->w0; level = lqr_owed_level(&root_of(c)->owed_inflate, level); }
+    return rc;
+}
 extern "C" int lqrhip_read_visible(LqrHipCarver *c, int w0, int h0, int w, int level, unsigned char *out)
 {
     int rc = batch_sync_of(c);
-    if (rc) return rc;
+    if (rc || (rc = read_visible_enter(c, w0, level))) return rc;
     size_t n = (size_t) w * h0 * px_bytes(c);
     Scratch tmp(g_stream0);
     uint8_t *d = tmp.get<uint8_t>(n, "&d", rc);
@@ -1631,7 +1753,7 @@
 extern "C" int lqrhip_read_visible_device(LqrHipCarver *c, int w0, int h0, int w, int level, void *device_out)
 {
     int rc = batch_sync_of(c);
-    if (rc) return rc;
+    if (rc || (rc = read_visible_enter(c, w0, level))) return rc;
     launch_read_visible(c, w0, h0, w, level, (uint8_t *) device_out);
     HIPCK(hipGetLastError());
     HIPCK(hipStreamSynchronize(g_stream0));
@@ -1642,7 +1764,7 @@
 extern "C" int lqrhip_read_sizes(LqrHipCarver *c, int w0, int h0, int transposed, const int *levels, int n, void *const *outs, int on_device)
 {
     int rc = batch_sync_of(c);
-    if (rc) return rc;
+    if (rc || (rc = owed_enter(c, LQR_OWED_AT_READ_SIZES))) return rc;
     if (n < 1 || !levels || !outs || w0 < 1 || h0 < 1) return LQRHIP_EARG;
     for (int k = 0; k < n; k++)
         if (levels[k] < 1 || levels[k] > w0 || !outs[k]) return LQRHIP_EARG;
@@ -1717,6 +1839,7 @@
 }
 extern "C" int lqrhip_discard_scan(LqrHipCarver *c, int w0, int h0, int w, int level, int depth, float strength, int which, int *out)
 {
+    if (c && !c->root) { const int paid = owed_enter(c, LQR_OWED_AT_DISCARD_SCAN); if (paid) return paid; }
     if (!c || c->root || !out || w0 < 1 || h0 < 1 || w < 1 || w > w0 || level < 1 || depth < 0 || !(which & 3) || !(strength >= 0.0f) || c->w0 != w0 || c->h0 != h0) {
         g_err = "discard scan: a root carver in its own base layout, a level, a strength >= 0 and a scan to run";
         return LQRHIP_EARG;
@@ -1772,6 +1895,14 @@
     return 0;
 }
 
+static int map_build_enter(LqrHipCarver *const *cs, int n)
+{
+    for (int i = 0; i < n; i++) {
+        int rc;
+        if (cs[i] && !cs[i]->root && (rc = owed_enter(cs[i], LQR_OWED_AT_MAP_BUILD))) return rc;
+    }
+    return 0;
+}
 struct __attribute__((visibility("hidden"))) LqrHipForward {
     struct Planes {
         DevBuf<float> in, p;
@@ -1821,6 +1952,7 @@
 {
     if (out) *out = nullptr;
     if (!cs || !out || n < 1 || n > LQRHIP_FORWARD_MAX_LINES || (orientation != 0 && orientation != 1) || w_start < 1) { g_err = "forward map: arguments"; return LQRHIP_EARG; }
+    { const int rc = map_build_enter(cs, n); if (rc) return rc; }
     const LqrHipCarver *c0 = cs[0];
     for (int i = 0; i < n; i++) {
         const LqrHipCarver *c = cs[i];
@@ -1904,7 +2036,7 @@
 {
     if (!c || c->root || !out || (orientation != 0 && orientation != 1)) return LQRHIP_EARG;
     int rc = batch_sync_of(c);
-    if (rc) return rc;
+    if (rc || (rc = owed_enter(c, LQR_OWED_AT_MAP_BUILD))) return rc;
     const int strided = (transposed != 0) != (orientation != 0);
     const int L = strided ? c->h0 : c->w0, H = strided ? c->w0 : c->h0;
     if (L > LQRHIP_MAX_FRAME_WIDTH || H > LQRHIP_FORWARD_MAX_LINES) return LQRHIP_EARG;
@@ -1942,6 +2074,7 @@
         g_err = "static energy: arguments";
         return LQRHIP_EARG;
     }
+    { const int rc = map_build_enter(cs, n); if (rc) return rc; }
     const LqrHipCarver *c0 = cs[0];
     for (int i = 0; i < n; i++) {
         const LqrHipCarver *c = cs[i];
@@ -2046,6 +2179,7 @@
         g_err = "clip forward map: arguments";
         return LQRHIP_EARG;
     }
+    { const int rc = map_build_enter(cs, n); if (rc) return rc; }
     const LqrHipCarver *c0 = cs[0];
     for (int i = 0; i < n; i++) {
         const LqrHipCarver *c = cs[i];
@@ -2180,8 +2314,12 @@
 
 extern "C" int lqrhip_read_vmap(LqrHipCarver *c, int w0, int h0, int w, int level, int depth, int *out)
 {
-    int rc = batch_sync_of(c);
-    if (rc) return rc;
+    int rc = batch_sync_of(c), act;
+    if (rc || (rc = owed_enter(c, LQR_OWED_AT_READ_VMAP, level, 0, &act))) return rc;
+    if (act == LQR_OWED_TRANSLATE) {
+        const LqrOwed &o = root_of(c)->owed_inflate;
+        w0 = c->w0; level = lqr_owed_level(&o, level); depth -= lqr_owed_seams(&o);
+    }
     size_t n = (size_t) w * h0;
     Scratch tmp(g_stream0);
     int32_t *d = tmp.get<int32_t>(n, "&d", rc);
@@ -2242,6 +2380,7 @@
     if (c->wk.bias || c->wk.rig) { free_working(c); c->stride = 0; c->wk_h = 0; }
     c->w0 = w; c->h0 = h;
     drop_catchup(c);
+    (void) owed_enter(c, LQR_OWED_AT_RESET);
     if ((rc = c->rgb0.alloc(n * px_bytes(c), "&c->rgb0")) || (rc = c->vs.alloc(n, "&c->vs"))) return rc;
     return 0;
 }
diff --git a/gimp-lqr-plugin_amd/host/lqr_carver.c b/gimp-lqr-plugin_amd/host/lqr_carver.c
--- a/gimp-lqr-plugin_amd/host/lqr_carver.c
+++ b/gimp-lqr-plugin_amd/host/lqr_carver.c
@@ -806,8 +806,13 @@
     HIP_ALL(g, lqrhip_batch_sync(B));
     HIP_ALL(g, lqrhip_vs_commit(B, r0->geo.w0, r0->geo.h0, s->wc0, s->n_seams, s->first_level, s->finish));
     for (i = 0; i < g->n; i++) (void) lqr_state_phase(&g->r[i]->state, LQR_STATE_INFLATING);
-    HIP_ALL(g, lqrhip_inflate(B, r0->geo.w0, r0->geo.h0, s->depth - 1, s->max_level));
-    HIP_ALL(g, lqrhip_planes_commit(B));
+    if (lqrhip_get_inflate_lazy()) {
+        HIP_ALL(g, lqrhip_levels_check(B, r0->geo.w0, r0->geo.h0, s->depth - 1, s->max_level));
+        HIP_ALL(g, lqrhip_inflate_owe(B, r0->geo.w0, r0->geo.h0, s->depth - 1, s->max_level));
+    } else {
+        HIP_ALL(g, lqrhip_inflate(B, r0->geo.w0, r0->geo.h0, s->depth - 1, s->max_level));
+        HIP_ALL(g, lqrhip_planes_commit(B));
+    }
     T_END(T_TAIL);
     FOR_TREE(g, i, r, {
         lqr_geom_session_done(&r->geo, s->depth, s->n_seams);
@@ -1465,6 +1470,7 @@
         CANCEL_POINT(g);
         if (s.transpose) LQR_CATCH(group_transpose(g));
         LQR_CATCH(group_build_maps(g, s.depth));
+        if (s.new_w > r->geo.w_start) HIP_ALL(g, lqrhip_inflate_pay(B));
         for (i = 0; i < g->n; i++) {
             set_width_tree(g->r[i], s.new_w);
             g->r[i]->session_rescale_current = walk.total - (s.gamma > 0 ? s.gamma : -s.gamma);
diff --git a/gimp-lqr-plugin_amd/host/lqr_owed.c b/gimp-lqr-plugin_amd/host/lqr_owed.c
--- /dev/null
+++ b/gimp-lqr-plugin_amd/host/lqr_owed.c
@@ -0,0 +1,39 @@
+#include "lqr_owed.h"
+
+int lqr_owed_any(const LqrOwed *o) { return o->max_level > 0; }
+int lqr_owed_seams(const LqrOwed *o) { return lqr_owed_any(o) ? o->l - o->max_level + 1 : 0; }
+int lqr_owed_depth(const LqrOwed *o) { return o->l + 1; }
+int lqr_owed_level(const LqrOwed *o, int level) { return level - lqr_owed_seams(o); }
+
+enum { BY_LEVEL = 16, BY_SESSION = 17 };
+static const unsigned char k_action[LQR_OWED_ENTRIES] = {
+    [LQR_OWED_AT_READ_VISIBLE] = BY_LEVEL,
+    [LQR_OWED_AT_FLATTEN] = BY_LEVEL,
+    [LQR_OWED_AT_COMMIT_FLAT] = LQR_OWED_DROP,
+    [LQR_OWED_AT_TRANSPOSE] = LQR_OWED_PAY,
+    [LQR_OWED_AT_RESET] = LQR_OWED_DROP,
+    [LQR_OWED_AT_ROLLBACK] = BY_SESSION,
+    [LQR_OWED_AT_WK_INIT] = LQR_OWED_PAY,
+    [LQR_OWED_AT_SESSION] = LQR_OWED_PAY,
+    [LQR_OWED_AT_INFLATE] = LQR_OWED_PAY,
+    [LQR_OWED_AT_READ_SIZES] = LQR_OWED_PAY,
+    [LQR_OWED_AT_READ_VMAP] = BY_LEVEL,
+    [LQR_OWED_AT_DISCARD_SCAN] = LQR_OWED_PAY,
+    [LQR_OWED_AT_ATTACH] = LQR_OWED_PAY,
+    [LQR_OWED_AT_ACTIVATE] = LQR_OWED_PAY,
+    [LQR_OWED_AT_MASK_WRITE] = LQR_OWED_PAY,
+    [LQR_OWED_AT_MASK_READ] = LQR_OWED_PAY,
+    [LQR_OWED_AT_MAP_BUILD] = LQR_OWED_PAY,
+    [LQR_OWED_AT_WIDTH] = LQR_OWED_PAY,
+};
+
+int lqr_owed_action(const LqrOwed *o, int entry, int level, int first_level)
+{
+    int a;
+    if (!lqr_owed_any(o)) return LQR_OWED_IGNORE;
+    if (entry < 0 || entry >= LQR_OWED_ENTRIES) return LQR_OWED_PAY;
+    a = k_action[entry];
+    if (a == BY_LEVEL) return level >= lqr_owed_depth(o) ? LQR_OWED_TRANSLATE : LQR_OWED_PAY;
+    if (a == BY_SESSION) return first_level == 2 * o->max_level - 1 ? LQR_OWED_DROP : LQR_OWED_IGNORE;
+    return a;
+}
diff --git a/gimp-lqr-plugin_amd/host/lqr_owed.h b/gimp-lqr-plugin_amd/host/lqr_owed.h
--- /dev/null
+++ b/gimp-lqr-plugin_amd/host/lqr_owed.h
@@ -0,0 +1,52 @@
+#ifndef LQR_OWED_H
+#define LQR_OWED_H
+
+#ifdef __cplusplus
+extern "C" {
+#endif
+
+enum {
+    LQR_OWED_AT_READ_VISIBLE = 0,
+    LQR_OWED_AT_FLATTEN,
+    LQR_OWED_AT_COMMIT_FLAT,
+    LQR_OWED_AT_TRANSPOSE,
+    LQR_OWED_AT_RESET,
+    LQR_OWED_AT_ROLLBACK,
+    LQR_OWED_AT_WK_INIT,
+    LQR_OWED_AT_SESSION,
+    LQR_OWED_AT_INFLATE,
+    LQR_OWED_AT_READ_SIZES,
+    LQR_OWED_AT_READ_VMAP,
+    LQR_OWED_AT_DISCARD_SCAN,
+    LQR_OWED_AT_ATTACH,
+    LQR_OWED_AT_ACTIVATE,
+    LQR_OWED_AT_MASK_WRITE,
+    LQR_OWED_AT_MASK_READ,
+    LQR_OWED_AT_MAP_BUILD,
+    LQR_OWED_AT_WIDTH,
+    LQR_OWED_ENTRIES
+};
+
+enum {
+    LQR_OWED_IGNORE = 0,
+    LQR_OWED_PAY = 1,
+    LQR_OWED_DROP = 2,
+    LQR_OWED_TRANSLATE = 3
+};
+
+typedef struct LqrOwed {
+    int l, max_level;
+} LqrOwed;
+
+int lqr_owed_any(const LqrOwed *o);
+int lqr_owed_seams(const LqrOwed *o);
+int lqr_owed_depth(const LqrOwed *o);
+
+int lqr_owed_action(const LqrOwed *o, int entry, int level, int first_level);
+int lqr_owed_level(const LqrOwed *o, int level);
+
+#ifdef __cplusplus
+}
+#endif
+
+#endif
diff --git a/include/lqr_hip.h b/include/lqr_hip.h
--- a/include/lqr_hip.h
+++ b/include/lqr_hip.h
@@ -89,6 +89,12 @@
 unsigned long long lqrhip_debug_pool_live(void);
 void lqrhip_debug_fixedcost(unsigned long long out4[4], int reset);
 int lqrhip_inflate(LqrHipBatch *b, int w0, int h0, int l, int max_level);
+int lqrhip_levels_check(LqrHipBatch *b, int w0, int h0, int l, int max_level);
+int lqrhip_inflate_owe(LqrHipBatch *b, int w0, int h0, int l, int max_level);
+int lqrhip_inflate_pay(LqrHipBatch *b);
+void lqrhip_set_inflate_lazy(int mode);
+int lqrhip_get_inflate_lazy(void);
+unsigned long long lqrhip_inflate_launches(int reset);
 typedef struct LqrHipVMap LqrHipVMap;
 int lqrhip_vmap_stage(const int *map, int on_device, int width, int height, int depth, int orientation, LqrHipVMap **out);
 int lqrhip_vmap_load(LqrHipBatch *b, const LqrHipVMap *m);
```

Result: no change. 630,300 Mseams*px/s, median of 6 (+1.1%).
